# NethermindEth/latticefold

Measured on AMD Instinct MI355X. Metric: folding-prover steps/sec (one NIFSProver::prove per step), GoldilocksRingNTT, higher is better.
Workload: dtype u64; 1 GPU; C4: GoldilocksRingNTT R1CS->CCS, m=N=2^20 rows, wit_len=262144, L=4, B=2^16, b=2, K=16, kappa=26, t=3; parallelism=replicas x1

## Files before the change

latticefold_amd/csrc/lf_capi.cpp:

```cpp
#include "lf_ring_host.h"
#include <thread>
#include <vector>

const char *lf_strerror(int code) {
    switch (code) {
        case LF_OK: return "ok";
        case LF_ERR_INVALID: return "invalid argument / wrong length";
        case LF_ERR_HIP: return "HIP runtime error (no GPU or out of device memory)";
        case LF_ERR_UNSUPPORTED: return "unsupported parameter";
        case LF_ERR_BAD_TABLES: return "ring tables are not a ring isomorphism";
        case LF_ERR_NORM: return "witness coefficient exceeds the decomposition bound";
        case LF_ERR_SIZE_BOUNDS: return "invalid size bounds (m must be >= wit_len*L, power of two)";
        case LF_ERR_STATE: return "call sequence misuse";
        case LF_ERR_REJECT: return "verifier rejected the proof";
    }
    return "unknown error";
}
const char *lf_phase_name(int i) { return (i >= 0 && i < LF_N_PHASES) ? PHASE_NAMES[i] : ""; }

static int install_tables(lf_ctx *c, u64 nonres, const u64 *y) {
    CrtTables T;
    if (build_crt_tables(nonres, y, T) != 0) return LF_ERR_BAD_TABLES;
    c->ring.T = T;
    c->dcrt = make_dev_crt(T);
// ... 524 lines not shown
            return hipGetLastError() == hipSuccess ? LF_ERR_UNSUPPORTED : LF_ERR_HIP;
    }
    c->ev_end(ev);
    launch_crt_fwd(c->dcrt, coef, ntt, ne, c->stream());
    launch_soa_to_aos(ntt, out_dev, ne, c->stream());
    if (hipGetLastError() != hipSuccess) return LF_ERR_HIP;
    return LF_OK;
}
int sb_cut_parts(lf_ctx *c, const lf_witness *wit, const char *name, const unsigned char **D) {
    const lf_params &P = c->P;
    if (!sb_base_ok(P.b) || c->sh_world > 1 || c->comm[0].model) return LF_ERR_UNSUPPORTED;
    if (!sb_digits_cover(P.b, P.K, P.B, c->digit_mode)) return LF_ERR_UNSUPPORTED;
    unsigned char *d;
    const size_t ldn = sb_ld(c->N);
    RET(c->tbuf(name, (size_t)P.K * 24 * ldn, &d));
    if (launch_sb_cut(wit->planes, c->N, P.K, sb_log2(P.b), c->digit_mode, d, ldn, c->stream()) != 0) return LF_ERR_HIP;
    *D = d;
    return LF_OK;
}
int commit_download(lf_ctx *c, const u64 *dev, size_t words, u64 *host) {
    RET(exchange_modsum_dev(c, (u64 *)dev, words));
    return down_small(c, dev, words, host);
}
void shard_slice(const lf_ctx *c, size_t n, size_t *i0, size_t *cnt) {
    size_t per = (n + (size_t)c->sh_world - 1) / (size_t)c->sh_world;
    size_t lo = per * (size_t)c->sh_rank;
    if (lo > n) lo = n;
    *i0 = lo;
    *cnt = lo + per > n ? n - lo : per;
}
bool shard_keep(const lf_ctx *c, int kind, size_t n) {
    const size_t Gw = (size_t)c->sh_world;
    if (Gw <= 1 || n / 2 < Gw * 64) return false;
    size_t thr = kind ? c->tn.shard_fold_min : c->tn.shard_lin_min;
    if (thr > (c->m >> 4)) thr = c->m >> 4;
    return n > thr;
}
int gather_slices(lf_ctx *c, u64 *buf, size_t planes, size_t n) {
    const size_t Gw = (size_t)c->sh_world, lcl = n / Gw, words = planes * lcl;
    u64 *gall, *gtmp;
    RET(c->tbuf("sh_gather_tab", words * Gw, &gall));
    RET(c->tbuf("sh_gather_tmp", words, &gtmp));
    HIPCHK(hipMemcpy2DAsync(gtmp, lcl * 8, buf + (size_t)c->sh_rank * lcl, n * 8, lcl * 8, planes, hipMemcpyDeviceToDevice, c->stream()));
    RET(c->cm().allgather_dev(gtmp, gall, words, c->stream()));
    launch_gather_relayout(gall, (u32)Gw, planes, lcl, buf, c->stream());
    return LF_OK;
}
int gather_parts(lf_ctx *c, const GatherPart *parts, int np, size_t lcl) {
    const size_t Gw = (size_t)c->sh_world;
    size_t ptot = 0;
    for (int i = 0; i < np; i++) ptot += parts[i].planes;
    const size_t words = ptot * lcl;
    u64 *gall, *gtmp;
    RET(c->tbuf("sh_gather_tab", words * Gw, &gall));
    RET(c->tbuf("sh_gather_tmp", words, &gtmp));
    size_t p0 = 0;
    for (int i = 0; i < np; i++) {
        HIPCHK(hipMemcpy2DAsync(gtmp + p0 * lcl, lcl * 8, parts[i].src, parts[i].src_ld * 8, lcl * 8, parts[i].planes, hipMemcpyDeviceToDevice, c->stream()));
        p0 += parts[i].planes;
    }
    RET(c->cm().allgather_dev(gtmp, gall, words, c->stream()));
    p0 = 0;
    for (int i = 0; i < np; i++) {
        launch_gather_relayout_part(gall, (u32)Gw, ptot, p0, parts[i].planes, lcl, parts[i].dst, c->stream());
        p0 += parts[i].planes;
    }
    return LF_OK;
}
int lf_ajtai_commit(lf_ctx *c, const uint64_t *f, size_t n, size_t batch, uint64_t *out) {
    if (LF_XB(c) && f && out) {
        XB x(c, true);
        int rc = lf_ajtai_commit(c, f, n, batch, out);
        if (rc == LF_OK) x.ring_out(out, batch * c->core_any().kappa);
        return rc;
    }
    if (!c || !f || !out || !batch) return LF_ERR_INVALID;
    return c->bb ? ring_ops<BbRing>::ajtai_commit(c->bb->p, f, n, batch, out) : ring_ops<GoldRing>::ajtai_commit(c, f, n, batch, out);
}
int lf_ajtai_commit_dev(lf_ctx *c, const uint64_t *f, size_t n, size_t batch, uint64_t *out) {
    if (!c || !f || !out || !batch) return LF_ERR_INVALID;
    if (LF_XB(c)) {
        XB x(c, true);
        int rc = lf_ajtai_commit_dev(c, f, n, batch, out);
        if (rc == LF_OK) x.ring_out(out, batch * c->core_any().kappa);
        return rc;
    }
    return c->bb ? ring_ops<BbRing>::ajtai_commit(c->bb->p, f, n, batch, out, Origin::device) : ring_ops<GoldRing>::ajtai_commit(c, f, n, batch, out, Origin::device);
}
static int ajtai_commit_gadget_api(lf_ctx *c, const uint64_t *f, bool ntt_in, size_t count, bool dec, uint64_t base, unsigned digits, size_t batch, uint64_t *out,
                                   Origin org = Origin::host) {
    if (LF_XB(c) && f && out) {
        XB x(c, true);
        const u32 kap = c->core_any().kappa;
        int rc = ajtai_commit_gadget_api(c, f, ntt_in, count, dec, base, digits, batch, out, org);
        if (rc == LF_OK) x.ring_out(out, batch * kap);
        return rc;
    }
    if (!c || !f || !out || !batch || digits == 0 || digits > 64) return LF_ERR_INVALID;
    u32 lb = 0;
    if (dec) {
        if (!pow2(base) || (c->bb && base > (1ull << 32))) return LF_ERR_UNSUPPORTED;
        while ((1ull << lb) < base) lb++;
    }
    return c->bb ? ring_ops<BbRing>::ajtai_commit_gadget(c->bb->p, f, ntt_in, count, lb, digits, batch, out, org)
                 : ring_ops<GoldRing>::ajtai_commit_gadget(c, f, ntt_in, count, lb, digits, batch, out, org);
}
int lf_ajtai_commit_coeff(lf_ctx *c, const uint64_t *f_coeff, size_t n, size_t batch, uint64_t *out) {
    return ajtai_commit_gadget_api(c, f_coeff, false, n, false, 0, 1, batch, out);
}
int lf_ajtai_decompose_and_commit_coeff(lf_ctx *c, const uint64_t *f_coeff, size_t count, uint64_t base, unsigned digits, size_t batch, uint64_t *out) {
    return ajtai_commit_gadget_api(c, f_coeff, false, count, true, base, digits, batch, out);
}
int lf_ajtai_decompose_and_commit_ntt(lf_ctx *c, const uint64_t *w_ntt, size_t count, uint64_t base, unsigned digits, size_t batch, uint64_t *out) {
    return ajtai_commit_gadget_api(c, w_ntt, true, count, true, base, digits, batch, out);
}
int lf_ajtai_commit_coeff_dev(lf_ctx *c, const uint64_t *f_coeff, size_t n, size_t batch, uint64_t *out) {
    return ajtai_commit_gadget_api(c, f_coeff, false, n, false, 0, 1, batch, out, Origin::device);
}
int lf_ajtai_decompose_and_commit_coeff_dev(lf_ctx *c, const uint64_t *f_coeff, size_t count, uint64_t base, unsigned digits, size_t batch, uint64_t *out) {
    return ajtai_commit_gadget_api(c, f_coeff, false, count, true, base, digits, batch, out, Origin::device);
}
int lf_ajtai_decompose_and_commit_ntt_dev(lf_ctx *c, const uint64_t *w_ntt, size_t count, uint64_t base, unsigned digits, size_t batch, uint64_t *out) {
    return ajtai_commit_gadget_api(c, w_ntt, true, count, true, base, digits, batch, out, Origin::device);
}

int lf_modsum(const uint64_t *parts, size_t nparts, size_t words, uint64_t *out) {
    if (!parts || !out || !nparts) return LF_ERR_INVALID;
    for (size_t w = 0; w < words; w++) {
        u64 acc = 0;
        for (size_t g = 0; g < nparts; g++) {
            u64 v = parts[g * words + w];
            if (v >= LF_P) return LF_ERR_INVALID;
            acc = fq_add(acc, v);
        }
        out[w] = acc;
    }
    return LF_OK;
}
int lf_modsum_ring(const uint64_t *parts, size_t nparts, size_t words, uint64_t *out, int ring) {
    if (ring == LF_RING_GOLDILOCKS) return lf_modsum(parts, nparts, words, out);
    if (ring != LF_RING_BABYBEAR || !parts || !out || !nparts) return LF_ERR_INVALID;
    for (size_t w = 0; w < words; w++) {
        u64 acc = 0;
        for (size_t g = 0; g < nparts; g++) {
            u64 v = parts[g * words + w];
            if (v >= lfbb::BB_P) return LF_ERR_INVALID;
            acc += v;
        }
        out[w] = acc % lfbb::BB_P;
    }
    return LF_OK;
}

int build_eq_dev(lf_ctx *c, const Fq3 *pt, u32 nv, u64 *eq_dev) {
    Fq3Const *rd;
    RET(c->tbuf("eq_point", 64, &rd));
    std::vector<Fq3Const> h(nv);
    for (u32 i = 0; i < nv; i++) h[i] = f3c(pt[i]);
    RET(c->h2d_small(rd, h.data(), nv * sizeof(Fq3Const)));
    if (nv >= 6) {
        u64 *scr;
        RET(c->tbuf("eq_scratch", build_eq_scratch_words(nv), &scr));
        launch_build_eq2(c->dcrt, rd, nv, scr, eq_dev, c->stream());
    } else launch_build_eq(c->dcrt, rd, nv, eq_dev, c->stream());
    return LF_OK;
}
static int build_eq_api(lf_ctx *c, const uint64_t *point, unsigned nv, uint64_t *out, Origin org) {
    if (LF_XB(c) && point && out && nv && nv <= 40) {
        XB x(c, org == Origin::device);
        int rc = build_eq_api(c, x.ext_in(point, nv), nv, out, org);
        if (rc == LF_OK && org == Origin::host) x.ext_out(out, (size_t)1 << nv);
        return rc;
    }
    if (!c || !point || !out || nv == 0 || nv > 40) return LF_ERR_INVALID;
    return c->bb ? ring_ops<BbRing>::build_eq(c->bb->p, point, nv, out, org) : ring_ops<GoldRing>::build_eq(c, point, nv, out, org);
}
int lf_build_eq(lf_ctx *c, const uint64_t *point, unsigned nv, uint64_t *out) { return build_eq_api(c, point, nv, out, Origin::host); }
int lf_build_eq_dev(lf_ctx *c, const uint64_t *point, unsigned nv, uint64_t *out) { return build_eq_api(c, point, nv, out, Origin::device); }
static int mle_eval_batch_api(lf_ctx *c, const uint64_t *tables, size_t ntables, size_t len, const uint64_t *point, unsigned nv, uint64_t *out, Origin org) {
    if (LF_XB(c) && tables && point && out) {
        XB x(c, true);
        int rc = mle_eval_batch_api(c, tables, ntables, len, x.ext_in(point, nv), nv, out, org);
        if (rc == LF_OK) x.ring_out(out, ntables);
        return rc;
    }
    if (!c || !tables || !point || !out || !ntables || nv == 0 || nv > 40) return LF_ERR_INVALID;
    return c->bb ? ring_ops<BbRing>::mle_eval_batch(c->bb->p, tables, ntables, len, point, nv, out, org)
                 : ring_ops<GoldRing>::mle_eval_batch(c, tables, ntables, len, point, nv, out, org);
}
int lf_mle_eval_batch(lf_ctx *c, const uint64_t *tables, size_t ntables, size_t len, const uint64_t *point, unsigned nv, uint64_t *out) {
    return mle_eval_batch_api(c, tables, ntables, len, point, nv, out, Origin::host);
}
int lf_mle_eval_batch_dev(lf_ctx *c, const uint64_t *tables, size_t ntables, size_t len, const uint64_t *point, unsigned nv, uint64_t *out) {
    return mle_eval_batch_api(c, tables, ntables, len, point, nv, out, Origin::device);
}

size_t lf_lcccs_len_ring(const lf_params *p, int ring) { return lcccs_len(p, ring == LF_RING_BABYBEAR ? 9 : 3); }
size_t lf_cccs_len_ring(const lf_params *p, int) { return cccs_len(p); }
size_t lf_proof_len_ring(const lf_params *p, int ring) { return proof_len(p, ring == LF_RING_BABYBEAR ? 9 : 3); }
size_t lf_lcccs_len(const lf_params *p) { return lcccs_len(p, 3); }
size_t lf_cccs_len(const lf_params *p) { return cccs_len(p); }
size_t lf_proof_len(const lf_params *p) { return proof_len(p, 3); }

int lf_ccs_load(lf_ctx *c, const lf_params *p, const uint32_t *const *rowptr, const uint32_t *const *col, const uint64_t *const *val,
                const uint32_t *S_off, const uint32_t *S_idx, const uint64_t *cc) {
    if (LF_XB(c) && p && rowptr && col && val && S_off && S_idx && cc && p->t >= 1 && p->t <= 8 && p->s <= 30 && p->q <= 8) {
        XB x(c);
        const size_t m = (size_t)1 << p->s;
        const uint64_t *v2[8];
        for (u32 j = 0; j < p->t; j++) {
            if (!rowptr[j] || !val[j]) return LF_ERR_INVALID;
            v2[j] = x.ring_in(val[j], rowptr[j][m]);
        }
        return lf_ccs_load(c, p, rowptr, col, v2, S_off, S_idx, x.ring_in(cc, p->q));
    }
    if (!c || !p || !rowptr || !col || !val || !S_off || !S_idx || !cc) return LF_ERR_INVALID;
    if (c->bb) { RET(lfbb::ccs_envelope(p)); return ring_ops<BbRing>::ccs_load(c->bb->p, p, rowptr, col, val, S_off, S_idx, cc); }
    if (p->s < 3 || p->s > LF_S_MAX || p->t == 0 || p->t > 8 || p->q == 0 || p->q > 8 || p->K == 0 || p->K > 32 || p->L == 0 || p->L > 8 ||
        p->d > 7 || p->wit_len == 0)
        return LF_ERR_UNSUPPORTED;
    if (p->b != 2 && !sb_base_ok(p->b)) return LF_ERR_UNSUPPORTED;
    if (p->b != 2 && (c->sh_world > 1 || c->comm[0].model || p->K > 11)) return LF_ERR_UNSUPPORTED;
    if (!pow2(p->B) || p->B > (1ULL << 32)) return LF_ERR_UNSUPPORTED;
    if (!sb_digits_cover(p->b, p->K, p->B, c->digit_mode)) return LF_ERR_UNSUPPORTED;
    return ring_ops<GoldRing>::ccs_load(c, p, rowptr, col, val, S_off, S_idx, cc);
}
int lf_spmv(lf_ctx *c, unsigned j, const uint64_t *z, uint64_t *out) {
    XbArrays xa(c);
    if (!c || !z || !out) return LF_ERR_INVALID;
    return c->bb ? ring_ops<BbRing>::spmv(c->bb->p, j, z, out) : ring_ops<GoldRing>::spmv(c, j, z, out);
}
int lf_spmv_dev(lf_ctx *c, unsigned j, const uint64_t *z, uint64_t *out) {
    if (!c || !z || !out) return LF_ERR_INVALID;
    XbArrays xa(c);
    return c->bb ? ring_ops<BbRing>::spmv(c->bb->p, j, z, out, Origin::device) : ring_ops<GoldRing>::spmv(c, j, z, out, Origin::device);
}

struct lf_witness_job {
    std::future<int> fut;
    lf_witness *w = nullptr;
};
int lf_witness_from_w_ccs_begin(lf_ctx *c, const uint64_t *w_ccs, lf_witness_job **job) {
    if (!c || !w_ccs || !job) return LF_ERR_INVALID;
    if (!c->have_ccs_any()) return LF_ERR_STATE;
    lf_witness_job *j = new lf_witness_job();
    c->io_jobs.fetch_add(1);
    j->fut = std::async(std::launch::async, [c, w_ccs, j]() -> int {
        struct Done { lf_ctx *c; ~Done() { c->io_jobs.fetch_sub(1); } } done{c};
        if (c->bb || c->xb.on) return lf_witness_from_w_ccs(c, w_ccs, &j->w);
        std::lock_guard<std::mutex> g(c->io_mu);
        if (hipSetDevice(c->device) != hipSuccess) return LF_ERR_HIP;
        t_lane = 2;
        return ring_ops<GoldRing>::witness_from_w_ccs_lane(c, w_ccs, &j->w);
    });
    *job = j;
    return LF_OK;
}
int lf_witness_job_finish(lf_witness_job *job, lf_witness **out) {
    if (!job) return LF_ERR_INVALID;
    const int rc = job->fut.valid() ? job->fut.get() : LF_ERR_STATE;
    if (rc == LF_OK && out) *out = job->w;
    else if (job->w) lf_witness_free(job->w);
    delete job;
    return rc;
}
int lf_witness_from_w_ccs(lf_ctx *c, const uint64_t *w_ccs, lf_witness **out) {
    XbArrays xa(c);
    if (!c || !w_ccs || !out) return LF_ERR_INVALID;
    return c->bb ? ring_ops<BbRing>::witness_from_w_ccs(c->bb->p, w_ccs, out) : ring_ops<GoldRing>::witness_from_w_ccs(c, w_ccs, out);
}
int lf_witness_from_f_coeff(lf_ctx *c, const uint64_t *f_coeff, lf_witness **out) {
    if (!c || !f_coeff || !out) return LF_ERR_INVALID;
    return c->bb ? ring_ops<BbRing>::witness_from_f_coeff(c->bb->p, f_coeff, out) : ring_ops<GoldRing>::witness_from_f_coeff(c, f_coeff, out);
}
int lf_witness_from_f(lf_ctx *c, const uint64_t *f_ntt, lf_witness **out) {
    XbArrays xa(c);
    if (!c || !f_ntt || !out) return LF_ERR_INVALID;
    return c->bb ? ring_ops<BbRing>::witness_from_f(c->bb->p, f_ntt, out) : ring_ops<GoldRing>::witness_from_f(c, f_ntt, out);
}
int lf_witness_get_f_coeff(lf_ctx *c, const lf_witness *w, uint64_t *out) {
    if (!c || !w || !out || w->ctx != c) return LF_ERR_INVALID;
    return c->bb ? ring_ops<BbRing>::witness_get_f_coeff(c->bb->p, w, out) : ring_ops<GoldRing>::witness_get_f_coeff(c, w, out);
}
int lf_witness_get_f(lf_ctx *c, const lf_witness *w, uint64_t *out) {
    XbArrays xa(c);
    if (!c || !w || !out || w->ctx != c) return LF_ERR_INVALID;
    return c->bb ? ring_ops<BbRing>::witness_get_f(c->bb->p, w, out) : ring_ops<GoldRing>::witness_get_f(c, w, out);
}
int lf_witness_get_w_ccs(lf_ctx *c, const lf_witness *w, uint64_t *out) {
    XbArrays xa(c);
    if (!c || !w || !out || w->ctx != c) return LF_ERR_INVALID;
    return c->bb ? ring_ops<BbRing>::witness_get_w_ccs(c->bb->p, w, out) : ring_ops<GoldRing>::witness_get_w_ccs(c, w, out);
}
int lf_witness_from_w_ccs_dev(lf_ctx *c, const uint64_t *w_ccs, lf_witness **out) {
    if (!c || !w_ccs || !out) return LF_ERR_INVALID;
    XbArrays xa(c);
    return c->bb ? ring_ops<BbRing>::witness_from_w_ccs(c->bb->p, w_ccs, out, Origin::device) : ring_ops<GoldRing>::witness_from_w_ccs(c, w_ccs, out, Origin::device);
}
int lf_witness_from_f_coeff_dev(lf_ctx *c, const uint64_t *f_coeff, lf_witness **out) {
    if (!c || !f_coeff || !out) return LF_ERR_INVALID;
    XbArrays xa(c);
    return c->bb ? ring_ops<BbRing>::witness_from_f_coeff(c->bb->p, f_coeff, out, Origin::device) : ring_ops<GoldRing>::witness_from_f_coeff(c, f_coeff, out, Origin::device);
}
int lf_witness_from_f_dev(lf_ctx *c, const uint64_t *f_ntt, lf_witness **out) {
    if (!c || !f_ntt || !out) return LF_ERR_INVALID;
    XbArrays xa(c);
    return c->bb ? ring_ops<BbRing>::witness_from_f(c->bb->p, f_ntt, out, Origin::device) : ring_ops<GoldRing>::witness_from_f(c, f_ntt, out, Origin::device);
}
int lf_witness_get_f_coeff_dev(lf_ctx *c, const lf_witness *w, uint64_t *out) {
    if (!c || !w || !out || w->ctx != c) return LF_ERR_INVALID;
    XbArrays xa(c);
    return c->bb ? ring_ops<BbRing>::witness_get_f_coeff(c->bb->p, w, out, Origin::device) : ring_ops<GoldRing>::witness_get_f_coeff(c, w, out, Origin::device);
}
int lf_witness_get_f_dev(lf_ctx *c, const lf_witness *w, uint64_t *out) {
    if (!c || !w || !out || w->ctx != c) return LF_ERR_INVALID;
    XbArrays xa(c);
    return c->bb ? ring_ops<BbRing>::witness_get_f(c->bb->p, w, out, Origin::device) : ring_ops<GoldRing>::witness_get_f(c, w, out, Origin::device);
// ... 243 lines not shown
```

latticefold_amd/csrc/lf_ctx.h:

```cpp
#pragma once
#include <hip/hip_runtime.h>
#include <assert.h>
#include <string.h>

#include <atomic>
#include <chrono>
#include <condition_variable>
#include <functional>
#include <future>
#include <thread>
#include <map>
#include <memory>
#include <mutex>
#include <set>
#include <string>
#include <vector>

#include "../../include/lfhip.h"
#include "bb_capi.h"
#include "lf_ctx_core.h"
#include "lf_common.h"
#include "lf_dist.h"
#include "lf_kernels.h"
#include "lf_sb.h"
// ... 3 lines not shown

namespace lf {
void launch_fix_many(const DevCrt &t, const u64 *in, size_t ld_in, u64 *out, size_t ld_out, size_t n_in, u32 rows3, Fq3Const r, hipStream_t s);
}

#include <stdio.h>
#include <stdlib.h>
static bool lf_trace_on() { static int v = -1; if (v < 0) v = getenv("LF_TRACE") ? 1 : 0; return v == 1; }
#define LF_TRACE(c, msg)                                                              \
    do {                                                                              \
        if (lf_trace_on()) {                                                          \
            hipError_t e_ = hipStreamSynchronize((c)->stream());                            \
            fprintf(stderr, "[lf] %s:%d %s -> %s\n", __func__, __LINE__, msg, hipGetErrorString(e_)); \
            fflush(stderr);                                                           \
        }                                                                             \
    } while (0)

inline thread_local int t_lane = 0;

struct lf_transcript {
    Transcript t;
    lfbb::BbTranscript *bb = nullptr;
    lf_transcript() {}
    lf_transcript(const lf_transcript &o) : t(o.t), bb(o.bb ? new lfbb::BbTranscript(*o.bb) : nullptr) {}
    ~lf_transcript() { delete bb; }
};

struct Timeline {
    bool on;
    std::chrono::steady_clock::time_point t0;
    std::vector<std::pair<const char *, double>> marks, marks1;
    Timeline() : on(getenv("LF_TIMELINE") != nullptr), t0(std::chrono::steady_clock::now()) { marks1.reserve(32); }
    void mark(const char *what) {
        marks.push_back({what, std::chrono::duration<double, std::milli>(std::chrono::steady_clock::now() - t0).count()});
    }
    void mark1(const char *what) { marks1.push_back({what, std::chrono::duration<double, std::milli>(std::chrono::steady_clock::now() - t0).count()}); }
    void merge() {
        marks.insert(marks.end(), marks1.begin(), marks1.end());
        marks1.clear();
        std::stable_sort(marks.begin(), marks.end(), [](const std::pair<const char *, double> &a, const std::pair<const char *, double> &b) { return a.second < b.second; });
    }
    void dump() {
        if (!on) return;
        double prev = 0;
        for (auto &m : marks) { fprintf(stderr, "[timeline] %-28s at %8.3f ms  (+%7.3f)\n", m.first, m.second, m.second - prev); prev = m.second; }
    }
};
inline thread_local Timeline *t_tl = nullptr;
#define TL_MARK(x) do { if (t_tl) t_tl->mark(x); } while (0)
inline const char *tl_round_name(const char *what, unsigned round) {
    static std::mutex mu;
    static std::set<std::string> names;
    char nm[32];
    snprintf(nm, sizeof nm, "%s %u", what, round);
    std::lock_guard<std::mutex> g(mu);
    return names.insert(nm).first->c_str();
}
#define TL_MARK_ROUND(what, round) do { if (t_tl) t_tl->mark(tl_round_name(what, round)); } while (0)

static const char *PHASE_NAMES[LF_N_PHASES] = {"linearization", "decomp_crt_commit", "decomp_evals", "fold_prepare",
                                                "fold_sumcheck", "fold_finish", "host_transcript", "total"};

struct LaneWorker {
    std::thread th;
    std::mutex m;
    std::condition_variable cv;
    std::function<int()> job;
    bool has_job = false, done = false, stop = false;
    int rc = 0;
    void loop() {
        std::unique_lock<std::mutex> lk(m);
        for (;;) {
            cv.wait(lk, [&] { return has_job || stop; });
            if (stop) return;
            std::function<int()> j = std::move(job);
            has_job = false;
            lk.unlock();
            int r = j();
            lk.lock();
            rc = r;
            done = true;
            cv.notify_all();
        }
    }
    void submit(std::function<int()> j) {
        std::unique_lock<std::mutex> lk(m);
        if (!th.joinable()) th = std::thread([this] { loop(); });
        job = std::move(j);
        has_job = true;
        done = false;
        cv.notify_all();
    }
    int wait() {
        std::unique_lock<std::mutex> lk(m);
        cv.wait(lk, [&] { return done; });
        return rc;
    }
    ~LaneWorker() {
        {
            std::unique_lock<std::mutex> lk(m);
            stop = true;
            cv.notify_all();
        }
        if (th.joinable()) th.join();
    }
};

struct lf_ctx : CtxCore<u64> {
    lf_ctx() : CtxCore<u64>(8192, 2 * 9 * 24 * sizeof(u64)) {}
    int lane() const override { return t_lane; }
    lfbb::BbCtx *bb = nullptr;
    ExtBasis xb;
    hipStream_t &st_io = st_lane[2];
    std::mutex io_mu;
    std::atomic<int> io_jobs{0};
    inline CtxCoreBase &core_any();
    bool have_ccs_any() { return core_any().have_ccs; }
    const lf_params &params_any() { return core_any().P; }
    size_t n_any() { return core_any().n; }
    size_t m_any() { return core_any().m; }
    size_t N_any() { return core_any().N; }
    HostRing ring;
    DevCrt dcrt;
    LaneWorker lane1;
    int agreed_two_lanes = -1;
    bool two_lanes_ok = false;
    lfdist::Comm comm[2];
    lfdist::Comm &cm() { assert(t_lane < 2); return comm[t_lane]; }
    bool ccs_general = false;
    size_t shc_r0 = (size_t)-1, shc_rcnt = 0, shc_lo = 0, shc_hi = 0;
    LinCombDesc desc{};
    std::vector<std::pair<const char *, double>> tl_marks;
    const lf_witness *bits_wit[2] = {nullptr, nullptr};
    u32 *bits_ptr[2] = {nullptr, nullptr};
    hipEvent_t bits_ev[2] = {nullptr, nullptr};
    hipEvent_t ev_yR = nullptr, ev_yL = nullptr;
    u64 *h_pin2 = nullptr;
    size_t h_pin2_words = 0;
    int pin2(size_t words) {
        if (words <= h_pin2_words) return LF_OK;
        if (h_pin2) (void)hipHostFree(h_pin2);
        h_pin2 = nullptr; h_pin2_words = 0;
        if (hipHostMalloc((void **)&h_pin2, words * 8) != hipSuccess) return LF_ERR_HIP;
        h_pin2_words = words;
        return LF_OK;
    }
    hipStream_t st_aux = nullptr;
    hipEvent_t ev_aux = nullptr;
    u64 *h_aux = nullptr;
    unsigned lin_split_rounds = 0;

    unsigned char *stage[LF_NLANES] = {nullptr, nullptr, nullptr};
    size_t stage_off[LF_NLANES] = {0, 0, 0};
    static constexpr size_t STAGE_BYTES = (size_t)1 << 20;
    int h2d_small(void *dst, const void *src, size_t bytes) {
        unsigned char *&ring = stage[t_lane];
        if (!ring && hipHostMalloc((void **)&ring, STAGE_BYTES, hipHostMallocDefault) != hipSuccess) { ring = nullptr; return LF_ERR_HIP; }
        const size_t need = (bytes + 63) & ~(size_t)63;
        if (need > STAGE_BYTES) {
            HIPCHK(hipMemcpyAsync(dst, src, bytes, hipMemcpyHostToDevice, stream()));
            HIPCHK(hipStreamSynchronize(stream()));
            return LF_OK;
        }
        if (stage_off[t_lane] + need > STAGE_BYTES) {
            HIPCHK(hipStreamSynchronize(stream()));
            stage_off[t_lane] = 0;
        }
        unsigned char *slot = ring + stage_off[t_lane];
        stage_off[t_lane] += need;
        memcpy(slot, src, bytes);
        HIPCHK(hipMemcpyAsync(dst, slot, bytes, hipMemcpyHostToDevice, stream()));
        return LF_OK;
    }
    TailMail *tail_mail = nullptr;
    u32 *tail_counters = nullptr;
    u64 *tail_dev_chal = nullptr;
    u32 tail_epoch = 0;
    int num_cus = 0;
    int tail_setup() {
        if (tail_mail) return LF_OK;
        hipDeviceProp_t pr;
        HIPCHK(hipGetDeviceProperties(&pr, device));
        num_cus = pr.multiProcessorCount;
        void *d = nullptr;
        HIPCHK(lf_dev_malloc(&d, 4096));
        HIPCHK(hipMemset(d, 0, 4096));
        tail_counters = (u32 *)d;
        tail_dev_chal = (u64 *)((char *)d + 1024);
        HIPCHK(hipHostMalloc((void **)&tail_mail, sizeof(TailMail), hipHostMallocMapped | hipHostMallocCoherent));
        memset(tail_mail, 0, sizeof(TailMail));
        return LF_OK;
    }
    u64 *d_poseidon = nullptr;
    int poseidon_setup() {
        if (d_poseidon) return LF_OK;
        const u64 *a, *m;
        Transcript::params(&a, &m);
        HIPCHK(lf_dev_malloc(&d_poseidon, (720 + 576) * 8));
        HIPCHK(hipMemcpy(d_poseidon, a, 720 * 8, hipMemcpyHostToDevice));
        HIPCHK(hipMemcpy(d_poseidon + 720, m, 576 * 8, hipMemcpyHostToDevice));
        return LF_OK;
    }
    hipEvent_t ev_theta = nullptr;
    hipEvent_t ev_block = nullptr;
    int lane_sync() {
        if (t_lane == 1 && ev_block) {
            HIPCHK(hipEventRecord(ev_block, st_lane[1]));
            HIPCHK(hipEventSynchronize(ev_block));
            return LF_OK;
        }
        HIPCHK(hipStreamSynchronize(stream()));
        return LF_OK;
    }
};
inline CtxCoreBase &lf_ctx::core_any() { return bb ? bb->core() : *this; }


#pragma GCC visibility push(hidden)
Fq3Const f3c(Fq3 a);
bool shard_keep(const lf_ctx *c, int kind, size_t n);
int build_eq_dev(lf_ctx *c, const Fq3 *pt, u32 nv, u64 *eq_dev);
int exchange_modsum_dev(lf_ctx *c, u64 *inout_dev, size_t words);
int down_small(lf_ctx *c, const u64 *dsrc, size_t words, u64 *host);
void shard_slice(const lf_ctx *c, size_t n, size_t *i0, size_t *cnt);
struct GatherPart { const u64 *src; size_t src_ld; u64 *dst; size_t planes; };
int shard_col_range(lf_ctx *c, size_t r0, size_t rcnt, size_t *lo, size_t *hi);
int gather_slices(lf_ctx *c, u64 *buf, size_t planes, size_t n);
struct SideState {
    const int32_t *planes = nullptr;
    u64 *z = nullptr;
    u64 *eq_r = nullptr;
    std::vector<u64> lcccs;
    std::atomic<int> z_state{0};
    hipEvent_t z_ev = nullptr;
    const unsigned char *D = nullptr;
    u32 *sv_bits = nullptr;
    ~SideState() { if (z_ev) (void)hipEventDestroy(z_ev); }
};
int gather_parts(lf_ctx *c, const GatherPart *parts, int np, size_t lcl);
inline thread_local bool t_xb_active = false;
inline thread_local bool t_xb_arrays = false;
struct XB {
    lf_ctx *c;
    size_t RE, TAU;
    std::vector<std::unique_ptr<std::vector<u64>>> keep;
    lf_transcript *tr = nullptr;
    explicit XB(lf_ctx *cc, bool arrays = false) : c(cc), RE((size_t)lf_ring_words(lf_ctx_ring(cc))), TAU((size_t)lf_ring_tau(lf_ctx_ring(cc))) {
        t_xb_active = true;
        t_xb_arrays = arrays;
    }
    ~XB() {
        t_xb_active = false;
        t_xb_arrays = false;
        if (tr) { tr->t.set_basis(nullptr, nullptr); if (tr->bb) tr->bb->set_basis(nullptr, nullptr); }
    }
    const u64 *ring_in(const u64 *p, size_t elems) {
        if (!p) return p;
        keep.emplace_back(new std::vector<u64>(p, p + elems * RE));
        c->xb.to_int(keep.back()->data(), elems * 8);
        return keep.back()->data();
    }
    const u64 *ext_in(const u64 *p, size_t n) {
        if (!p) return p;
        keep.emplace_back(new std::vector<u64>(p, p + n * TAU));
        c->xb.to_int(keep.back()->data(), n);
        return keep.back()->data();
    }
    void ring_out(u64 *p, size_t elems) { if (p) c->xb.to_ext(p, elems * 8); }
    void ext_out(u64 *p, size_t n) { if (p) c->xb.to_ext(p, n); }
    void transcript(lf_transcript *t) {
        tr = t;
        if (t->bb) t->bb->set_basis(c->xb.T, c->xb.Ti);
        else t->t.set_basis(c->xb.T, c->xb.Ti);
    }
};
#define LF_XB(c) ((c) && (c)->xb.on && !t_xb_active)
struct XbArrays {
    const bool set;
    explicit XbArrays(lf_ctx *c) : set(LF_XB(c)) { if (set) t_xb_active = t_xb_arrays = true; }
    ~XbArrays() { if (set) t_xb_active = t_xb_arrays = false; }
};
int fold_impl(lf_ctx *c, Transcript &tr, SideState *S , u64 *lcccs_out, lf_witness **w_out, u64 *proof);
int commit_download(lf_ctx *c, const u64 *dev, size_t words, u64 *host);
int commit_parts_i8g(lf_ctx *c, const unsigned char *D, size_t ldn, u32 NP, u64 *out_dev);
int sb_cut_parts(lf_ctx *c, const lf_witness *wit, const char *name, const unsigned char **D);
int fold_impl_sb(lf_ctx *c, Transcript &tr, SideState *S , u64 *lcccs_out, lf_witness **w_out, u64 *proof);
struct FoldStep {
    lf_ctx *c;
    Transcript &tr;
    SideState *S;
    u64 *proof;
    const lf_params &P;
    const size_t m, n, N;
    const u32 K, K2, deg;
    const GoldV hv;
    std::vector<Fq3> alpha, zeta, mu, beta, pt;
    Fq3Const *d_mu = nullptr, *d_ap = nullptr, *d_zp = nullptr;
    u64 *G[2] = {nullptr, nullptr}, *eqb = nullptr, *zz = nullptr;
    FoldRoundArgs a;
    u64 *T5[2] = {nullptr, nullptr};
    const u64 *curF = nullptr;
    size_t ldF = 0;
    u64 *eq0 = nullptr, *q = nullptr, *dpart = nullptr, *d_theta = nullptr, *d_eta = nullptr;
    FoldStep(lf_ctx *c, Transcript &tr, SideState *S, u64 *proof);
    u64 *msg(u32 round) const { return proof + (size_t)(round - 1) * (deg + 1) * 24; }
    u64 *theta() const { return proof + (size_t)P.s * (deg + 1) * 24; }
    u64 *eta() const { return theta() + (size_t)K2 * 72; }
    int powers_alpha_zeta();
    int powers_mu();
    int prepare_buffers();
    int side_mz(int sd, hipStream_t st, u64 *zb, const char *zaos_name, size_t zc_lo, size_t zc_hi, size_t g_r0 = 0, size_t g_rcnt = (size_t)-1);
    void first_tables();
    void fix_special(u32 round, Fq3Const r, u64 *dst, hipStream_t sg);
    void set_tables(u64 *dst, size_t nn);
    int eval_buffers();
    int gather_q(hipStream_t s1f);
    int finish(u64 *lcccs_out, lf_witness **w_out, const std::function<int(const std::vector<int8_t> &rho8, int8_t *d_rho, int32_t *npl)> &fold_witness);
};
int sb_fold_round_abi(lf_ctx *c, const u64 *t5, const u64 *F, size_t n, const Fq3Const *d_mu, u64 *evals_out);
int dot_batch_dev(lf_ctx *c, const u64 *X, size_t ldx, u32 na, const u64 *Y, size_t ldy, u32 nb, size_t n, u64 *dpart, u64 *od, hipStream_t st = nullptr,
                         const char *tag = "", unsigned char *yb_pre = nullptr);
int coef_eval_dev(lf_ctx *c, const int32_t *planes, size_t n, const u64 *eq, size_t ldeq, u32 K, int mode_bits, u64 *partial, u64 *od, size_t ldp,
                         const lf_witness *wit = nullptr);
int lin_tail_rounds(lf_ctx *c, Transcript &tr, const u64 *cur, const u64 *cure, size_t n, u64 *tout, u64 *partial, u32 round, Fq3 *point,
                           u64 *msgs, u32 deg, const std::function<void(u32)> *after_round);
int build_z(lf_ctx *c, const int32_t *planes, u32 K, int mode_bits, const u64 *heads, u64 *z, size_t w0 = 0, size_t wcnt = (size_t)-1,
            const unsigned char *D = nullptr );
#pragma GCC visibility pop
```

latticefold_amd/csrc/lf_fold.cpp:

```cpp
#include "lf_ring_host.h"

static int tail_host_rounds(lf_ctx *c, Transcript &tr, u32 epoch, u32 nr, u32 npts, bool dev_transcript, u64 *msgs, Fq3 *pt,
                            const std::function<void(u32)> *after_round = nullptr, u32 round0 = 0) {
    TailMail *mail = c->tail_mail;
    const auto t_start = std::chrono::steady_clock::now();
    double host_us = 0, wait_us = 0;
    auto t_mark = t_start;
    const bool tl_on = t_tl && t_tl->on;
    for (u32 i = 0; i < nr; i++) {
        u32 spins = 0;
        while (__atomic_load_n(&mail->msg_seq[i], __ATOMIC_ACQUIRE) != epoch) {
            __builtin_ia32_pause();
            if ((++spins & 0xfff) == 0) {
                if (__atomic_load_n(&mail->err, __ATOMIC_RELAXED) == epoch ||
                    std::chrono::duration<double>(std::chrono::steady_clock::now() - t_start).count() > 10.0) {
                    __atomic_store_n(&mail->abort_seq, epoch, __ATOMIC_RELEASE);
                    (void)hipStreamSynchronize(c->stream());
                    return LF_ERR_HIP;
                }
            }
        }
        if (tl_on) { auto nw = std::chrono::steady_clock::now(); wait_us += std::chrono::duration<double, std::micro>(nw - t_mark).count(); t_mark = nw; }
        u64 *evs = msgs + (size_t)i * npts * 24;
        memcpy(evs, (const void *)mail->msg[i], (size_t)npts * 24 * 8);
        HostTimer ht(c);
        Fq3 r;
        if (dev_transcript) r = fq3_make(mail->chal_out[i][0], mail->chal_out[i][1], mail->chal_out[i][2]);
        else r = lfs::sumcheck_round<GoldV>(tr, evs, npts);
        pt[i] = r;
        if (i + 1 < nr && !dev_transcript) {
            mail->chal[i][0] = r.c[0]; mail->chal[i][1] = r.c[1]; mail->chal[i][2] = r.c[2];
            __atomic_store_n(&mail->chal_seq[i], epoch, __ATOMIC_RELEASE);
        }
        if (after_round) (*after_round)(round0 + i);
        if (tl_on) { auto nw = std::chrono::steady_clock::now(); host_us += std::chrono::duration<double, std::micro>(nw - t_mark).count(); t_mark = nw; }
    }
    if (dev_transcript) tr.set_state((const u64 *)mail->sponge);
    if (tl_on) fprintf(stderr, "[timeline]    tail: %u rounds, host transcript %.1f us, waiting for the GPU %.1f us\n", nr, host_us, wait_us);
    return LF_OK;
}
static int tail_sponge_to_device(lf_ctx *c, Transcript &tr, u64 **state_out) {
    RET(c->poseidon_setup());
    *state_out = c->tail_dev_chal + 4 * TAIL_MAX_ROUNDS;
    u64 st[26];
    tr.get_state(st);
    HIPCHK(hipMemcpyAsync(*state_out, st, sizeof(st), hipMemcpyHostToDevice, c->stream()));
    HIPCHK(hipStreamSynchronize(c->stream()));
    return LF_OK;
}
int lin_tail_rounds(lf_ctx *c, Transcript &tr, const u64 *cur, const u64 *cure, size_t n, u64 *tout, u64 *partial, u32 round, Fq3 *point,
                           u64 *msgs, u32 deg, const std::function<void(u32)> *after_round) {
    const lf_params &P = c->P;
    RET(c->tail_setup());
    LinTailArgs A;
    A.T = cur; A.E = cure; A.Tout = tout; A.n0 = n; A.rounds = P.s - round + 1; A.deg = deg; A.partial = partial;
    RET(c->tbuf("lin_tail_priv", lin_tail_priv_words(n, P.t), &A.priv));
    A.counters = c->tail_counters; A.dev_chal = c->tail_dev_chal;
    HIPCHK(hipHostGetDevicePointer((void **)&A.mail, c->tail_mail, 0));
    if (++c->tail_epoch >= (1u << 30)) c->tail_epoch = 1;
    A.epoch = c->tail_epoch;
    A.r_first = f3c(point[round - 2]);
    A.dev_transcript = (c->tn.device_transcript && !c->xb.on) ? 1u : 0u;
    A.pos_ark = A.pos_mds = nullptr; A.sponge_state = nullptr;
    if (A.dev_transcript) {
        RET(tail_sponge_to_device(c, tr, &A.sponge_state));
        A.pos_ark = c->d_poseidon; A.pos_mds = c->d_poseidon + 720;
    }
    if (launch_lin_tail(c->dcrt, c->desc, A, c->stream()) == 0) return LF_ERR_UNSUPPORTED;
    if (hipGetLastError() != hipSuccess) return LF_ERR_HIP;
    return tail_host_rounds(c, tr, A.epoch, A.rounds, deg + 1, A.dev_transcript != 0, msgs + (size_t)(round - 1) * (deg + 1) * 24, &point[round - 1], after_round, round);
}
static int fold_tail_rounds(lf_ctx *c, Transcript &tr, const FoldRoundArgs &a, u64 *curF, u64 *const Fbuf[2], u64 *T_other, const Fq3Const *d_mu,
                            u64 *partial, u32 round, std::vector<Fq3> &pt, u64 *msgs, u32 deg) {
    const lf_params &P = c->P;
    RET(c->tail_setup());
    const u32 nr = P.s - round + 1;
    FoldTailArgs A;
    A.T[0] = (u64 *)a.eqL; A.T[1] = T_other;
    A.F[0] = curF; A.F[1] = curF == Fbuf[0] ? Fbuf[1] : Fbuf[0];
    A.n0 = a.n; A.rounds = nr; A.K = P.K; A.mu_pow = d_mu; A.partial = partial;
    A.counters = c->tail_counters; A.dev_chal = c->tail_dev_chal;
    RET(c->tbuf("tail_eqpriv", fold_tail_eqpriv_words(a.n, P.K), &A.eqpriv));
    HIPCHK(hipHostGetDevicePointer((void **)&A.mail, c->tail_mail, 0));
    if (++c->tail_epoch >= (1u << 30)) c->tail_epoch = 1;
    A.epoch = c->tail_epoch;
    A.r_first = f3c(pt[round - 2]);
    A.dev_transcript = (c->tn.device_transcript && !c->xb.on) ? 1u : 0u;
    A.pos_ark = A.pos_mds = nullptr; A.sponge_state = nullptr;
    if (A.dev_transcript) {
        RET(tail_sponge_to_device(c, tr, &A.sponge_state));
        A.pos_ark = c->d_poseidon; A.pos_mds = c->d_poseidon + 720;
    }
    if (launch_fold_tail(c->dcrt, A, c->num_cus, c->stream()) == 0) return LF_ERR_UNSUPPORTED;
    if (hipGetLastError() != hipSuccess) return LF_ERR_HIP;
    return tail_host_rounds(c, tr, A.epoch, nr, deg + 1, A.dev_transcript != 0, msgs + (size_t)(round - 1) * (deg + 1) * 24, &pt[round - 1]);
}

FoldStep::FoldStep(lf_ctx *c_, Transcript &tr_, SideState *S_, u64 *proof_)
    : c(c_), tr(tr_), S(S_), proof(proof_), P(c_->P), m(c_->m), n(c_->n), N(c_->N), K(c_->P.K), K2(2 * c_->P.K), deg(2 * c_->P.b), hv{c_->ring}, pt(c_->P.s) {}
int FoldStep::powers_alpha_zeta() {
    std::vector<Fq3Const> a_pow((size_t)K2 * 3), z_pow((size_t)K2 * P.t);
    for (u32 i = 0; i < K2; i++) {
        lfs::powers(hv, alpha[i], 3, [&](u32 d, const Fq3 &pw) { a_pow[(size_t)i * 3 + d] = f3c(pw); });
        lfs::powers(hv, zeta[i], P.t, [&](u32 j, const Fq3 &pw) { z_pow[(size_t)i * P.t + j] = f3c(pw); });
    }
    RET(upload_consts(c, "c_ap", a_pow, &d_ap));
    return upload_consts(c, "c_zp", z_pow, &d_zp);
}
int FoldStep::powers_mu() {
    std::vector<Fq3Const> mu_pow((size_t)K2 * 3);
    for (u32 i = 0; i < K2; i++) lfs::powers(hv, mu[i], 3, [&](u32 d, const Fq3 &pw) { mu_pow[(size_t)i * 3 + d] = f3c(pw); });
    return upload_consts(c, "c_mu", mu_pow, &d_mu);
}
int FoldStep::prepare_buffers() {
    RET(c->tbuf("fold_G1", 24 * m, &G[0]));
    RET(c->tbuf("fold_G2", 24 * m, &G[1]));
    RET(c->tbuf("fold_eqb", 3 * m, &eqb));
    return c->tbuf("fold_zz", (size_t)P.t * 24 * n, &zz);
}
int FoldStep::side_mz(int sd, hipStream_t st, u64 *zb, const char *zaos_name, size_t zc_lo, size_t zc_hi, size_t g_r0, size_t g_rcnt) {
    launch_lincomb_z(c->dcrt, S[sd].z + zc_lo, n, K, d_zp + (size_t)sd * K * P.t, P.t, zc_hi - zc_lo, zb + zc_lo, st);
    if (c->ccs_general) {
        u64 *zaos;
        RET(c->tbuf(zaos_name, (size_t)P.t * n * 24, &zaos));
        launch_spmv_rows(c->dcrt, P.t, c->d_rowptr.data(), c->d_col.data(), c->d_val.data(), zb, (size_t)24 * n, n, zaos, G[sd], m, 0, st, g_r0, g_rcnt);
    } else
        launch_spmv_sum(c->dcrt, P.t, c->d_rowptr.data(), c->d_col.data(), c->d_val.data(), zb, (size_t)24 * n, n, G[sd], m, st, g_r0, g_rcnt);
    return LF_OK;
}
void FoldStep::first_tables() {
    a.eqL = S[0].eq_r; a.eqR = S[1].eq_r; a.eqB = eqb; a.G1 = G[0]; a.G2 = G[1]; a.ld = m; a.n = m;
    a.p0 = 0; a.pcnt = m / 2; a.pF0 = 0;
}
void FoldStep::set_tables(u64 *dst, size_t nn) {
    a.eqL = dst; a.eqR = dst + 3 * nn; a.eqB = dst + 6 * nn; a.G1 = dst + 9 * nn; a.G2 = dst + 33 * nn;
    a.ld = nn; a.n = nn;
}
void FoldStep::fix_special(u32 round, Fq3Const r, u64 *dst, hipStream_t sg) {
    const size_t nn = a.n / 2;
    if (round == 2) {
        launch_fix_many(c->dcrt, a.eqL, a.ld, dst, nn, a.n, 1, r, sg);
        launch_fix_many(c->dcrt, a.eqR, a.ld, dst + 3 * nn, nn, a.n, 1, r, sg);
        launch_fix_many(c->dcrt, a.eqB, a.ld, dst + 6 * nn, nn, a.n, 1, r, c->stream());
        launch_fix_many(c->dcrt, a.G1, a.ld, dst + 9 * nn, nn, a.n, 8, r, sg);
        launch_fix_many(c->dcrt, a.G2, a.ld, dst + 33 * nn, nn, a.n, 8, r, sg);
    } else if (sg != c->stream()) {
        launch_fix_many(c->dcrt, a.eqL, a.ld, dst, nn, a.n, 2, r, sg);
        launch_fix_many(c->dcrt, a.eqB, a.ld, dst + 6 * nn, nn, a.n, 1, r, c->stream());
        launch_fix_many(c->dcrt, a.G1, a.ld, dst + 9 * nn, nn, a.n, 16, r, sg);
    } else {
        launch_fix_many(c->dcrt, a.eqL, a.ld, dst, nn, a.n, 19, r, c->stream());
    }
}
int FoldStep::eval_buffers() {
    u64 *fsm;
    RET(c->tbuf("fold_eq0", 3 * m, &eq0));
    RET(c->tbuf("dec_q", (size_t)P.t * 24 * n, &q));
    RET(c->tbuf("dot_partial", dot_partial_words(K, P.t), &dpart));
    RET(c->tbuf("fold_small", (size_t)K2 * 72 + (size_t)K2 * P.t * 24 + 64, &fsm));
    d_theta = fsm; d_eta = fsm + (size_t)K2 * 72;
    return build_eq_dev(c, pt.data(), P.s, eq0);
}
int FoldStep::gather_q(hipStream_t s1f) {
    size_t c0, cnt;
    shard_slice(c, n, &c0, &cnt);
    if (P.t > 1) RET(c->fork(c->stream(), s1f));
    for (u32 j = 0; j < P.t; j++)
        launch_spmv_t_eq(c->dcrt, c->d_colptr[j], c->d_rowidx[j], c->d_valT[j], eq0, m, q + (size_t)j * 24 * n, n, (j & 1) ? s1f : c->stream(), c0, cnt);
    if (P.t > 1) RET(c->join(s1f, c->stream()));
    return LF_OK;
}
int FoldStep::finish(u64 *lcccs_out, lf_witness **w_out, const std::function<int(const std::vector<int8_t> &, int8_t *, int32_t *)> &fold_witness) {
    std::vector<u64> rho_c, rho;
    std::vector<int8_t> rho8;
    {
        HostTimer ht(c);
        tr.absorb_ring(eta(), (size_t)K2 * P.t);
        lfs::draw_rho(hv, tr, K2, rho_c, rho, &rho8);
    }
    int8_t *d_rho;
    RET(c->tbuf("c_rho", (size_t)K2 * 24 + 64, &d_rho));
    int32_t *npl;
    RET(lf_planes_alloc(c, N * 24 * 4, &npl));
    RET(fold_witness(rho8, d_rho, npl));
    u64 *nf = nullptr, *nw = nullptr;
    const size_t nf_bytes = N * 24 * 8, nw_bytes = (size_t)P.wit_len * 24 * 8;
    RET(lf_planes_alloc(c, nf_bytes, (int32_t **)&nf));
    RET(lf_planes_alloc(c, nw_bytes, (int32_t **)&nw));
    launch_recompose_crt(c->dcrt, npl, N, (u32)N, 1, P.B, 1, 0, nf, N, 0, c->stream());
    launch_recompose_crt(c->dcrt, npl, N, P.wit_len, P.L, P.B, 1, 0, nw, P.wit_len, 0, c->stream());
    if (hipGetLastError() != hipSuccess) return LF_ERR_HIP;
    LF_TRACE(c, "fold_witness");
    TL_MARK("  eta absorbed, rho drawn, fold_witness enqueued");
    {
        HostTimer ht(c);
        const size_t ll = lf_lcccs_len(&P);
        lfs::fold_instance(hv, P, pt, theta(), eta(), rho_c.data(), rho.data(), [&](u32 i) { return &S[i / K].lcccs[(size_t)(i % K) * ll * 24]; }, lcccs_out);
    }
    TL_MARK("  folded instance on the host");
    HIPCHK(hipStreamSynchronize(c->stream()));
    *w_out = new lf_witness{c, npl, N, c->device, N * 24 * 4};
    (*w_out)->f_ntt = nf; (*w_out)->f_bytes = nf_bytes; (*w_out)->w_ccs = nw; (*w_out)->w_bytes = nw_bytes;
    TL_MARK(" rho + fold_witness");
    return LF_OK;
}
static void fold_tab_poly(const GoldV &hv, u32 round, const Fq3 &r1v, std::vector<u64> &poly) {
    const int nd = round == 1 ? 2 : 4, ncode = round == 1 ? 9 : 81;
    poly.assign((size_t)ncode * 12, 0);
    const Fq3 one = fq3_one();
    auto small = [&](int v) { return v == 0 ? fq3_zero() : (v > 0 ? (v == 1 ? one : fq3_add(one, one)) : (v == -1 ? fq3_neg(one) : fq3_neg(fq3_add(one, one)))); };
    for (int code = 0; code < ncode; code++) {
        int dg[4] = {0, 0, 0, 0}, cc = code;
        for (int b = 0; b < nd; b++, cc /= 3) dg[b] = cc % 3 - 1;
        Fq3 f0, f1;
        if (round == 1) { f0 = small(dg[0]); f1 = small(dg[1]); }
        else {
            f0 = fq3_add(small(dg[0]), hv.ext_mul(small(dg[1] - dg[0]), r1v));
            f1 = fq3_add(small(dg[2]), hv.ext_mul(small(dg[3] - dg[2]), r1v));
        }
        Fq3 df = fq3_sub(f1, f0), f0s = hv.ext_mul(f0, f0), dfs = hv.ext_mul(df, df);
        Fq3 t1 = hv.ext_mul(f0s, df), t2 = hv.ext_mul(f0, dfs);
        Fq3 q[4] = {fq3_sub(hv.ext_mul(f0s, f0), f0), fq3_sub(fq3_add(fq3_add(t1, t1), t1), df), fq3_add(fq3_add(t2, t2), t2), hv.ext_mul(dfs, df)};
        for (int e = 0; e < 4; e++)
            for (int w = 0; w < 3; w++) poly[(size_t)code * 12 + 3 * e + w] = q[e].c[w];
    }
}
struct FoldB2 : FoldStep {
    using FoldStep::FoldStep;
    const size_t Gw = (size_t)c->sh_world, gr = (size_t)c->sh_rank;
    bool sv_split = false, fr_split = false, fused = false, use_lut = false, use_r4tab = false, use_r5 = false, use_sv = false, sv_two_streams = false;
    bool sharded = false;
    int flip = 0, fmode = 0;
    const u64 *prevF = nullptr;
    size_t prevld = 0, ldEr = 0;
    u64 *svE[3] = {nullptr, nullptr, nullptr}, *svE_rest = nullptr;
    u32 svE_level = 1;
    lfs::SplitCoef<GoldV> sp{};
    bool split_now = false;
    const u64 *Er = nullptr;
    u64 *F[2] = {nullptr, nullptr}, *partial = nullptr, *od = nullptr, *od_host = nullptr, *od_shard = nullptr, *d_lut = nullptr;
    u32 *sv_bits[2] = {nullptr, nullptr};
    hipStream_t sv_g_stream = nullptr;

    u64 *svE_ptr(u32 l) const {
        if (l <= 3) return svE[l - 1];
        size_t off = 0;
        for (u32 q = 4; q < l; q++) off += 3 * (m >> q);
        return svE_rest + off;
    }
    void svE_ensure(u32 l) {
        for (; svE_level < l; svE_level++)
            launch_eq_pairsum(svE_ptr(svE_level), m >> svE_level, m >> (svE_level + 1), svE_ptr(svE_level + 1), m >> (svE_level + 1), c->stream());
    }
    int prepare(), rounds_begin(), tail_handoff(u32 round, bool *done), fix_tables(u32 round, u64 *dst, bool *gathered), choose_producer(u32 round);
    void decide_split(u32 round);
    int gemm_round(u32 round), dispatch(u32 round), collect(u32 round), rounds(), evaluations();
};

int FoldB2::prepare() {
    { HostTimer ht(c); lfs::draw_alpha_zeta<GoldV>(tr, K2, alpha, zeta); }
    size_t ph = c->ev_begin(13);
    RET(powers_alpha_zeta());
    RET(prepare_buffers());
    RET(c->tbuf("round_partial", round_partial_words(), &partial));
    od = od_host = c->round_out();
    if (!od) return LF_ERR_HIP;
    if (c->sh_world > 1) {
        RET(c->tbuf("fold_round_out", 5 * 24 + 8, &od_shard));
        od = od_shard;
    }
    const bool shard_tabs = shard_keep(c, 1, m);
    const size_t g_r0 = shard_tabs ? (size_t)c->sh_rank * (m / (size_t)c->sh_world) : 0, g_rcnt = shard_tabs ? m / (size_t)c->sh_world : (size_t)-1;
    size_t zc_lo = 0, zc_hi = n;
    if (shard_tabs) RET(shard_col_range(c, g_r0, g_rcnt, &zc_lo, &zc_hi));
    {
        hipStream_t s0 = c->stream(), s1 = (t_lane == 0) ? c->st_lane[1] : s0;
        u64 *zz1 = zz;
        if (s1 != s0) RET(c->tbuf("fold_zz1", (size_t)P.t * 24 * n, &zz1));
        RET(c->fork(s0, s1));
        for (int sd = 0; sd < 2; sd++) {
            hipStream_t st = sd ? s1 : s0;
            RET(side_mz(sd, st, sd ? zz1 : zz, sd ? "spmv_zaos_R" : "spmv_zaos_L", zc_lo, zc_hi, g_r0, g_rcnt));
            launch_add_fhat_comb(c->dcrt, S[sd].planes, N, K, d_ap + (size_t)sd * K * 3, G[sd], m, st, g_r0, g_rcnt);
        }
        RET(c->join(s1, s0));
    }
    { HostTimer ht(c); lfs::draw_mu_beta<GoldV>(tr, K2, P.s, mu, beta); }
    TL_MARK(" fold challenges");
    RET(powers_mu());
    RET(build_eq_dev(c, beta.data(), P.s, eqb));
    sv_split = !c->tn.fold_sv_no_split && P.s >= 4 && m >= 256;
    if (sv_split) {
        RET(c->tbuf("fold_svE1", 3 * (m / 2), &svE[0]));
        RET(c->tbuf("fold_svE2", 3 * (m / 4), &svE[1]));
        RET(c->tbuf("fold_svE3", 3 * (m / 8), &svE[2]));
        RET(build_eq_dev(c, beta.data() + 1, P.s - 1, svE[0]));
    }
    fr_split = sv_split && c->sh_world == 1 && c->dcrt.nu2p40 && !c->tn.fold_rounds_no_split;
    if (fr_split) RET(c->tbuf("fold_svE_rest", 3 * (m / 8) + 64, &svE_rest));
    LF_TRACE(c, "fold prepare");
    c->ev_end(ph);
    if (t_tl && t_tl->on) { (void)hipStreamSynchronize(c->stream()); TL_MARK(" fold prepare (synced)"); }
    return LF_OK;
}
int FoldB2::rounds_begin() {
    sharded = Gw > 1;
    fused = !c->tn.fold_unfused && (Gw == 1 || !c->tn.shard_plain_rounds);
    use_lut = fused && P.s >= 4 && m / 4 >= c->tn.lut_min && m / 4 >= 4 && !c->tn.fold_no_lut;
    use_r4tab = use_lut && c->dcrt.nu2p40 && !c->tn.fold_no_r4tab;
    use_r5 = use_r4tab && !c->tn.fold_no_r5tab && Gw == 1 && P.s >= 5 && (N & 3) == 0 && (c->tn.no_tail || m / 8 > c->tn.tail_n) && m / 32 >= c->tn.r5_min;
    const size_t half = m / 2, f0_ent = use_lut ? m / 16 : m / 4, f1_ent = use_r5 ? m / 32 : m / 8;
    RET(c->tbuf("fold_F0", (size_t)K2 * 3 * 24 * (f0_ent ? f0_ent : 1), &F[0]));
    RET(c->tbuf("fold_F1", (size_t)K2 * 3 * 24 * (f1_ent ? f1_ent : 1), &F[1]));
    RET(c->tbuf("fold_T0", 57 * (half ? half : 1), &T5[0]));
    RET(c->tbuf("fold_T1", 57 * (half / 2 ? half / 2 : 1), &T5[1]));
    first_tables();
    c->sv_round_mask = 0;
    c->fold_split_mask = 0;
    sv_two_streams = t_lane == 0 && Gw == 1;
    sv_g_stream = c->stream();
    use_sv = !c->tn.force_exchange && !c->tn.fold_no_sv && (Gw == 1 || !c->tn.shard_plain_rounds) && N <= m && (N & 3) == 0 && !c->tn.fold_tab_r1;
    return LF_OK;
}
int FoldB2::tail_handoff(u32 round, bool *done) {
    if (sharded || c->tn.no_tail || round < 5 || !curF || ldF != a.n || a.n > c->tn.tail_n || a.n < 4 || P.s - round + 1 > TAIL_MAX_ROUNDS) return LF_OK;
    int trc = fold_tail_rounds(c, tr, a, (u64 *)curF, F, T5[flip], d_mu, partial, round, pt, proof, deg);
    if (trc == LF_OK) {
        curF = (u64 *)curF == F[0] ? F[1] : F[0];
        ldF = 2;
        *done = true;
    }
    return trc == LF_ERR_UNSUPPORTED ? LF_OK : trc;
}
int FoldB2::fix_tables(u32 round, u64 *dst, bool *gathered) {
    const Fq3Const r = f3c(pt[round - 2]);
    const size_t nn = a.n / 2;
    const bool handover = sharded && !shard_keep(c, 1, nn);
    hipStream_t sg = c->stream();
    if (use_sv && sv_two_streams && !sharded && (int)round <= c->tn.sv_rounds && round <= 3 && nn / 2 >= c->tn.sv_min && sv_shape_ok(1 << (round - 1), nn / 2, K))
        sg = c->st_lane[1];
    sv_g_stream = sg;
    if (!sharded) { fix_special(round, r, dst, sg); return LF_OK; }
    const size_t j0 = gr * (nn / Gw), jc = nn / Gw;
    if (round == 2) {
        launch_fix_many(c->dcrt, a.eqL + 2 * j0, a.ld, dst + j0, nn, 2 * jc, 1, r, sg);
        launch_fix_many(c->dcrt, a.eqR + 2 * j0, a.ld, dst + 3 * nn + j0, nn, 2 * jc, 1, r, sg);
        launch_fix_many(c->dcrt, a.eqB + 2 * j0, a.ld, dst + 6 * nn + j0, nn, 2 * jc, 1, r, sg);
        launch_fix_many(c->dcrt, a.G1 + 2 * j0, a.ld, dst + 9 * nn + j0, nn, 2 * jc, 8, r, sg);
        launch_fix_many(c->dcrt, a.G2 + 2 * j0, a.ld, dst + 33 * nn + j0, nn, 2 * jc, 8, r, sg);
    } else {
        launch_fix_many(c->dcrt, a.eqL + 2 * j0, a.ld, dst + j0, nn, 2 * jc, 19, r, sg);
    }
    if (!handover) return LF_OK;
    sharded = false;
    if (round <= 3) return gather_slices(c, dst, 57, nn);
    u64 *fd = F[(round & 1) ? 0 : 1];
    const size_t lcl = ldF / 2;
    launch_fix_many(c->dcrt, curF, ldF, fd, lcl, ldF, K2 * 3 * 8, r, c->stream());
    const GatherPart gp[2] = {{dst + gr * lcl, nn, dst, 57}, {fd, lcl, fd, (size_t)K2 * 3 * 24}};
    RET(gather_parts(c, gp, 2, lcl));
    curF = fd; ldF = nn;
    *gathered = true;
    return LF_OK;
}
int FoldB2::choose_producer(u32 round) {
    const size_t nn = a.n / 2;
    if (round == 3) {
        const size_t q = sharded ? nn / Gw : nn, j0 = sharded ? gr * q : 0;
        if (use_lut) {
            Fq3 lut[162];
            lfs::fold_lut81(hv, pt[0], pt[1], lut);
            RET(c->tbuf("fold_lut", 2 * 81 * 3 + 8, &d_lut));
            RET(c->h2d_small(d_lut, lut, sizeof(lut)));
            fmode = 3;
            curF = nullptr; ldF = q;
        } else {
            Fq3 Wf[4];
            lfs::eq_weights(hv, pt.data(), 2, Wf);
            const Fq3Const W[4] = {f3c(Wf[0]), f3c(Wf[1]), f3c(Wf[2]), f3c(Wf[3])};
            launch_fold_materialize2(c->dcrt, S[0].planes, S[1].planes, N, j0, q, K, W, F[0], c->stream());
            curF = F[0]; ldF = q;
        }
    } else if (round > 3) {
        u64 *fd = F[(round & 1) ? 0 : 1];
        if (use_lut && round == 4) fmode = 4;
        else if (use_r5 && round == 5) fmode = 7;
        else if (fused && ldF >= c->tn.fuse_min && ldF >= 4) { prevF = curF; prevld = ldF; fmode = 1; }
        else launch_fix_many(c->dcrt, curF, ldF, fd, ldF / 2, ldF, K2 * 3 * 8, f3c(pt[round - 2]), c->stream());
        curF = fd; ldF = ldF / 2;
    }
    return LF_OK;
}
void FoldB2::decide_split(u32 round) {
    Er = nullptr; ldEr = 0; split_now = false;
    if (!(fr_split && round >= 2 && !sharded && (fmode == 7 || (fmode == 4 && use_r4tab)) && a.pcnt >= c->tn.fold_split_min)) return;
    sp = lfs::split_coef(hv, lfs::eq_prefix(hv, beta.data(), pt.data(), round), beta[round - 1]);
    if (!sp.ok) return;
    svE_ensure(round);
    Er = svE_ptr(round); ldEr = m >> round;
    split_now = true;
    c->fold_split_mask |= 1u << (round - 1);
}
int FoldB2::gemm_round(u32 round) {
    const int svV = 1 << (round - 1);
    std::vector<Fq3> W((size_t)svV), Cf;
    lfs::eq_weights(hv, pt.data(), round - 1, W.data());
    lfs::sv_coef(hv, svV, W.data(), sv_num_pairs(svV), [&](int i) { return sv_pair(svV, i); }, Cf);
    u64 *d_coef, *gtmp, *svtp;
    unsigned char *sveb;
    int32_t *svpart, *svtot;
    RET(c->tbuf("sv_coef", Cf.size() * 3 + 8, &d_coef));
    RET(c->tbuf("sv_gtmp", 128, &gtmp));
    RET(c->tbuf("sv_tp", sv_tp_words(K), &svtp));
    RET(c->tbuf("sv_eb", sv_eb_bytes(a.pcnt), &sveb));
    RET(c->tbuf("sv_part", sv_part_words(svV, a.pcnt, K), &svpart));
    RET(c->tbuf("sv_tot", sv_tot_words(svV, K), &svtot));
    RET(c->h2d_small(d_coef, Cf.data(), Cf.size() * sizeof(Fq3)));
    if (!sv_bits[0])
        for (int sd = 0; sd < 2; sd++) {
            if (S[sd].sv_bits) { sv_bits[sd] = S[sd].sv_bits; continue; }
            RET(c->tbuf(sd ? "sv_bits_R" : "sv_bits_L", sv_bits_words(N, K), &sv_bits[sd]));
            launch_sv_bits(S[sd].planes, N, N, K, sv_bits[sd], c->stream());
        }
    hipStream_t sg = round == 1 ? (sv_two_streams && !sharded ? c->st_lane[1] : c->stream()) : sv_g_stream;
    if (round == 1) RET(c->fork(c->stream(), sg));
    launch_fold_round_g(c->dcrt, a, partial, gtmp, sg);
    hipEvent_t g_ready = nullptr;
    if (sg != c->stream() && !(g_ready = c->join_mark(sg))) return LF_ERR_HIP;
    const u64 *Ei = nullptr;
    size_t ldE = 0;
    Fq3Const w01[2] = {};
    if (sv_split) {
        const Fq3 ci = lfs::eq_prefix(hv, beta.data(), pt.data(), round), bi = beta[round - 1];
        w01[0] = f3c(hv.ext_mul(ci, fq3_sub(fq3_one(), bi)));
        w01[1] = f3c(hv.ext_mul(ci, bi));
        svE_ensure(round);
        Ei = svE[round - 1]; ldE = m >> round;
    }
    if (launch_sv_round(c->dcrt, svV, sv_bits[0], sv_bits[1], N, a.eqB, a.ld, a.p0, a.pcnt, K, d_mu, d_coef, sveb, svpart, svtot, svtp, gtmp, od, c->stream(), g_ready,
                        Ei, ldE, w01) != 0)
        return LF_ERR_UNSUPPORTED;
    c->sv_round_mask |= 1u << (round - 1);
    return LF_OK;
}
int FoldB2::dispatch(u32 round) {
    const int32_t *pL = S[0].planes, *pR = S[1].planes;
    hipStream_t st = c->stream();
    if (use_sv && (int)round <= c->tn.sv_rounds && round <= 3 && a.pcnt >= c->tn.sv_min && sv_shape_ok(1 << (round - 1), a.pcnt, K) && (a.p0 * ((size_t)1 << (round - 1))) % 256 == 0)
        return gemm_round(round);
    if ((round == 2 || (round == 1 && c->tn.fold_tab_r1)) && a.pcnt >= c->tn.tab_min) {
        std::vector<u64> poly;
        fold_tab_poly(hv, round, round == 2 ? pt[0] : fq3_zero(), poly);
        u64 *d_poly, *d_tp;
        RET(c->tbuf("fold_poly", 81 * 12 + 8, &d_poly));
        RET(c->tbuf("fold_tp", (size_t)K2 * 3 * 81 * 12, &d_tp));
        RET(c->h2d_small(d_poly, poly.data(), poly.size() * 8));
        launch_fold_round_tab(c->dcrt, (int)round, a, pL, pR, N, K, d_mu, d_poly, d_tp, partial, od, st);
        return LF_OK;
    }
    if (round == 1) launch_fold_round1(c->dcrt, a, pL, pR, N, K, d_mu, partial, od, st);
    else if (round == 2) launch_fold_round2(c->dcrt, a, pL, pR, N, K, d_mu, f3c(pt[0]), partial, od, st);
    else if (fmode == 3 && c->dcrt.nu2p40) {
        u64 *mutab;
        RET(c->tbuf("fold_mutab", (size_t)3 * K2 * 3 * 81 * 4, &mutab));
        launch_fold_round_lut_mu(c->dcrt, a, pL, pR, N, d_lut, mutab, K, d_mu, partial, od, st);
    } else if (fmode == 3) launch_fold_round_lut(c->dcrt, a, pL, pR, N, d_lut, K, d_mu, partial, od, st);
    else if (fmode == 4 && use_r4tab) {
        u64 *r4sq, *r4mt;
        RET(c->tbuf("fold_r4sq", (size_t)6561 * 4, &r4sq));
        RET(c->tbuf("fold_r4mt", (size_t)K2 * 3 * 162 * 4, &r4mt));
        launch_fold_round_lut_fix_tab(c->dcrt, a, pL, pR, N, d_lut, f3c(pt[round - 2]), r4sq, r4mt, use_r5 ? nullptr : (u64 *)curF, ldF, K, d_mu, partial, od, st, Er, ldEr);
    } else if (fmode == 7) {
        u64 *r5xx, *r5yy, *r5mt;
        RET(c->tbuf("fold_r5xx", (size_t)6561 * 4, &r5xx));
        RET(c->tbuf("fold_r5yy", (size_t)6561 * 4, &r5yy));
        RET(c->tbuf("fold_r5mt", (size_t)K2 * 3 * 324 * 4, &r5mt));
        launch_fold_round_lut_fix5(c->dcrt, a, pL, pR, N, d_lut, f3c(pt[round - 3]), f3c(pt[round - 2]), r5xx, r5yy, r5mt, (u64 *)curF, ldF, K, d_mu, partial, od, st, Er, ldEr);
    } else if (fmode == 4) launch_fold_round_lut_fix(c->dcrt, a, pL, pR, N, d_lut, f3c(pt[round - 2]), (u64 *)curF, ldF, K, d_mu, partial, od, st);
    else if (fmode == 1) launch_fold_round_fix(c->dcrt, a, prevF, prevld, f3c(pt[round - 2]), (u64 *)curF, ldF, K, d_mu, partial, od, st, Er, ldEr);
    else launch_fold_round(c->dcrt, a, curF, ldF, K, d_mu, partial, od, st);
    if (split_now) {
        u64 *partial_g;
        RET(c->tbuf("round_partial_g", round_partial_words(), &partial_g));
        launch_fold_round_g(c->dcrt, a, partial_g, od + 120, st);
    }
    return LF_OK;
}
int FoldB2::collect(u32 round) {
    if (od == od_shard) {
        if (sharded) RET(exchange_modsum_dev(c, od, (size_t)(deg + 1) * 24));
        HIPCHK(hipMemcpyAsync(od_host, od, (size_t)(deg + 1) * 24 * 8, hipMemcpyDeviceToHost, c->stream()));
    }
    return c->lane_sync();
}
int FoldB2::rounds() {
    size_t ph = c->ev_begin(14);
    { HostTimer ht(c); lfs::sumcheck_prologue<GoldV>(tr, P.s, deg); }
    RET(rounds_begin());
    for (u32 round = 1; round <= P.s; round++) {
        fmode = 0;
        bool done = false;
        RET(tail_handoff(round, &done));
        if (done) break;
        if (round > 1) {
            const size_t nn = a.n / 2;
            u64 *dst = T5[flip];
            bool gathered = false;
            RET(fix_tables(round, dst, &gathered));
            if (!gathered) RET(choose_producer(round));
            set_tables(dst, nn);
            flip ^= 1;
        }
        if (sharded && !shard_keep(c, 1, a.n)) sharded = false;
        if (sharded) { a.pcnt = a.n / 2 / Gw; a.p0 = gr * a.pcnt; a.pF0 = a.p0; }
        else { a.p0 = 0; a.pcnt = a.n / 2; a.pF0 = 0; }
        decide_split(round);
        size_t ev = c->ev_begin(0);
        RET(dispatch(round));
        c->ev_end(ev);
        LF_TRACE(c, "fold round");
        RET(collect(round));
        u64 *evs = msg(round);
        if (split_now) {
            HostTimer ht2(c);
            lfs::complete_fold_split(hv, sp, od_host, od_host + 120, msg(round - 1), pt[round - 2], evs);
        } else
            memcpy(evs, od_host, (size_t)(deg + 1) * 24 * 8);
        HostTimer ht(c);
        pt[round - 1] = lfs::sumcheck_round<GoldV>(tr, evs, deg + 1);
        if (round <= 3 || round == 6 || round == 10) TL_MARK_ROUND("  round", round);
    }
    TL_MARK(" fold sumcheck");
    c->ev_end(ph);
    return LF_OK;
}
int FoldB2::evaluations() {
    u64 *red;
    RET(c->tbuf("red_partial", 256 * 4096, &red));
    RET(eval_buffers());
    hipStream_t s1 = (t_lane == 0 && c->sh_world == 1 && c->st_lane[1]) ? c->st_lane[1] : c->stream();
    RET(gather_q(s1));
    RET(c->pin((size_t)K2 * 72 + (size_t)K2 * P.t * 24));
    u64 *hp = c->h_pin_ref();
    if (P.s >= 4 && curF && ldF == 2 && !c->tn.theta_eval) launch_fix_final(c->dcrt, curF, K2 * 3 * 8, f3c(pt[P.s - 1]), d_theta, c->stream());
    else {
        size_t i0, cnt;
        shard_slice(c, N, &i0, &cnt);
        for (int sd = 0; sd < 2; sd++) RET(coef_eval_dev(c, S[sd].planes + i0, cnt, eq0 + i0, m, K, 1, red, d_theta + (size_t)sd * K * 72, N));
        RET(exchange_modsum_dev(c, d_theta, (size_t)K2 * 72));
    }
    HIPCHK(hipMemcpyAsync(hp, d_theta, (size_t)K2 * 72 * 8, hipMemcpyDeviceToHost, c->stream()));
    if (!c->ev_theta) HIPCHK(hipEventCreateWithFlags(&c->ev_theta, hipEventDisableTiming));
    HIPCHK(hipEventRecord(c->ev_theta, c->stream()));
    {
        size_t c0, cnt;
        shard_slice(c, n, &c0, &cnt);
        if (s1 != c->stream()) {
            unsigned char *ybq = nullptr;
            if (!c->tn.dot_valu && cnt >= c->tn.dot_min && P.t <= 3 && K <= 16 && ((((size_t)(S[0].z + c0)) ^ ((size_t)(S[1].z + c0))) & 15) == 0) {
                RET(c->tbuf("dot_yb", dot_i8_yb_bytes(n + 1), &ybq));
                if (launch_dot_pack_y(S[0].z + c0, q + c0, n, P.t, cnt, ybq, c->stream()) != 0) ybq = nullptr;
            }
            RET(c->fork(c->stream(), s1));
            u64 *dpart1;
            RET(c->tbuf("dot_partial1", dot_partial_words(K, P.t), &dpart1));
            RET(dot_batch_dev(c, S[1].z + c0, n, K, q + c0, n, P.t, cnt, dpart1, d_eta + (size_t)K * P.t * 24, s1, "_1", ybq));
            if (!c->join_mark(s1)) return LF_ERR_HIP;
            RET(dot_batch_dev(c, S[0].z + c0, n, K, q + c0, n, P.t, cnt, dpart, d_eta, nullptr, "", ybq));
            RET(c->join_wait(c->stream()));
        } else
            for (int sd = 0; sd < 2; sd++) RET(dot_batch_dev(c, S[sd].z + c0, n, K, q + c0, n, P.t, cnt, dpart, d_eta + (size_t)sd * K * P.t * 24));
        RET(exchange_modsum_dev(c, d_eta, (size_t)K2 * P.t * 24));
    }
    HIPCHK(hipMemcpyAsync(hp + (size_t)K2 * 72, d_eta, (size_t)K2 * P.t * 24 * 8, hipMemcpyDeviceToHost, c->stream()));
    HIPCHK(hipEventSynchronize(c->ev_theta));
    memcpy(theta(), hp, (size_t)K2 * 72 * 8);
    {
        HostTimer ht(c);
        tr.absorb_ring(theta(), (size_t)K2 * 3);
    }
    HIPCHK(hipStreamSynchronize(c->stream()));
    memcpy(eta(), hp + (size_t)K2 * 72, (size_t)K2 * P.t * 24 * 8);
    TL_MARK(" theta/eta");
    return LF_OK;
}
int fold_impl(lf_ctx *c, Transcript &tr, SideState *S , u64 *lcccs_out, lf_witness **w_out, u64 *proof) {
    if (c->P.b != 2) return fold_impl_sb(c, tr, S, lcccs_out, w_out, proof);
    FoldB2 f(c, tr, S, proof);
    RET(f.prepare());
    RET(f.rounds());
    size_t ph = c->ev_begin(15);
    RET(f.evaluations());
    RET(f.finish(lcccs_out, w_out, [&](const std::vector<int8_t> &rho8, int8_t *d_rho, int32_t *npl) -> int {
        HIPCHK(hipMemcpyAsync(d_rho, rho8.data(), rho8.size(), hipMemcpyHostToDevice, c->stream()));
        LF_TRACE(c, "theta/eta");
        launch_fold_witness(S[0].planes, S[1].planes, f.N, f.K, d_rho, npl, c->stream());
        return LF_OK;
    }));
    c->ev_end(ph);
    return LF_OK;
}

// ... 123 lines not shown
```

latticefold_amd/csrc/lf_kernels.h:

```cpp
#pragma once
#include "lf_ajtai_i8.h"
#include "lf_sv_rounds.h"
#include <hip/hip_runtime.h>

#include "lf_host.h"

namespace lf {

struct DevCrt {
    u64 nu;
    int nu2p40;
    u64 w4, w2, w10, w1, w7, w5, w11;
    int slot_of_pos[8], pos1[8], pos2[8];
    u64 tw1[8], tw2[8];
};
DevCrt make_dev_crt(const CrtTables &T);

struct Fq3Const { u64 c[3]; };

struct XbMat3 { u64 m[9]; };
void launch_aos_to_soa(const u64 *aos, u64 *soa, size_t n, hipStream_t s, u32 *flag = nullptr, const XbMat3 *Ti = nullptr);
void launch_soa_to_aos(const u64 *soa, u64 *aos, size_t n, hipStream_t s, const u32 *unless_flag = nullptr, const XbMat3 *T = nullptr);
void launch_ext_to_aos(const u64 *soa, u64 *aos, size_t n, hipStream_t s, const XbMat3 *T = nullptr);
void launch_slot_const_check(const u64 *tab, size_t n, u32 *flag, hipStream_t s);
void launch_fill_uniform(u64 *dst, size_t words, u64 seed, size_t start, hipStream_t s);
void launch_fill_ajtai(u64 *A, u32 kappa, size_t n, size_t n_total, size_t col0, u64 seed, hipStream_t s, u32 row0 = 0);

void launch_modsum(const u64 *parts, u32 nparts, size_t words, u64 *out, hipStream_t s);
void launch_gather_relayout(const u64 *all, u32 nranks, size_t planes, size_t lcl, u64 *full, hipStream_t s);
void launch_gather_relayout_part(const u64 *all, u32 nranks, size_t planes_tot, size_t p0, size_t planes, size_t lcl, u64 *full, hipStream_t s);

constexpr u32 SELFTEST_OUT = 13, SELFTEST_OUTC = 12;
void launch_selftest_field(const u64 *in, u32 n, u32 nc, u64 nu_gen, u64 *out, u64 *outc, u64 *mism_dev, hipStream_t s);

void launch_crt_fwd(const DevCrt &t, const u64 *coef, u64 *ntt, size_t n, hipStream_t s);
void launch_icrt_dense(const u64 *icrt_mat , const u64 *ntt, u64 *coef, size_t n, hipStream_t s);
void launch_ring_mul_ntt(const DevCrt &t, const u64 *a, const u64 *b, size_t n_terms, size_t n, u64 *out, hipStream_t s, u32 *flag = nullptr, const XbMat3 *Ti = nullptr);
void launch_ring_mul_coeff(const DevCrt &t, const u64 *icrt_mat , const u64 *a, const u64 *b, size_t n_terms, size_t n, u64 *out, hipStream_t s);


void launch_decompose(const u64 *coef, size_t n, u64 base, u32 digits, int layout, u64 *out, hipStream_t s, int mode = 0);
void launch_recompose(const u64 *in, size_t n_out, u64 base, u32 digits, u64 *out, hipStream_t s);
void launch_coef_to_i32(const u64 *coef, int32_t *planes, size_t n, u32 bound, int *viol, hipStream_t s);
void launch_i32_to_coef(const int32_t *planes, u64 *coef, size_t n, hipStream_t s);
void launch_recompose_crt(const DevCrt &t, const int32_t *planes, size_t n_planes, u32 wit_len, u32 L, u64 B, u32 K,
                          int mode_bits, u64 *out, size_t ldz, size_t off, hipStream_t s);
void launch_linf(const u64 *coef, size_t n, u64 *out_max, hipStream_t s);


void launch_build_eq(const DevCrt &t, const Fq3Const *r_dev , u32 nv, u64 *eq , hipStream_t s);
size_t build_eq_scratch_words(u32 nv);
void launch_build_eq2(const DevCrt &t, const Fq3Const *r_dev, u32 nv, u64 *scratch, u64 *eq, hipStream_t s);
void launch_spmv(const DevCrt &t, const u32 *rowptr, const u32 *col, const u64 *val , const u64 *z,
                 size_t ldz, u64 *out, size_t m, int accumulate, hipStream_t s, size_t r0 = 0, size_t rcnt = (size_t)-1 );
void launch_spmv_sum(const DevCrt &t, u32 nm, const u32 *const *rowptr, const u32 *const *col, const u64 *const *val, const u64 *z,
                     size_t z_stride, size_t ldz, u64 *out, size_t m, hipStream_t s, size_t r0 = 0, size_t rcnt = (size_t)-1 );
void launch_spmv_rows(const DevCrt &t, u32 nm, const u32 *const *rowptr, const u32 *const *col, const u64 *const *val, const u64 *z, size_t z_stride, size_t n,
                      u64 *zaos, u64 *out, size_t m, int accumulate, hipStream_t s, size_t r0 = 0, size_t rcnt = (size_t)-1);
void launch_spmv_t_eq(const DevCrt &t, const u32 *colptr, const u32 *rowidx, const u64 *val, const u64 *eq, size_t m,
                      u64 *q, size_t n, hipStream_t s, size_t c0 = 0, size_t ccnt = (size_t)-1 );
void launch_dot_batch(const DevCrt &t, const u64 *X, size_t ldx, u32 na, const u64 *Y, size_t ldy, u32 nb, size_t n,
                      u64 *partial, u64 *out, hipStream_t s);
size_t dot_partial_words(u32 na, u32 nb);
void launch_dot_eq(const DevCrt &t, const u64 *X, size_t ldx, u32 na, const u64 *eq, size_t ldeq, size_t n, u64 *partial,
                   u64 *out, hipStream_t s);
void launch_coef_eval(const DevCrt &t, const int32_t *planes, size_t n, const u64 *eq, size_t ldeq, u32 K, int mode_bits,
                      u64 *partial, u64 *out, hipStream_t s, size_t ldp = 0);
size_t coef_eval_partial_words(u32 K);
void launch_lincomb_z(const DevCrt &t, const u64 *z, size_t ldz, u32 K, const Fq3Const *coef_dev , u32 tt, size_t n,
                      u64 *out, hipStream_t s, u32 per_slot = 0);
void launch_add_fhat_comb(const DevCrt &t, const int32_t *planes, size_t n_planes, u32 K, const Fq3Const *apow_dev ,
                          u64 *G, size_t m, hipStream_t s, size_t r0 = 0, size_t rcnt = (size_t)-1 );

void launch_fix_ring(const DevCrt &t, const u64 *in, u64 *out, size_t n_in, Fq3Const r, hipStream_t s);
void launch_fix_fq3(const DevCrt &t, const u64 *in, u64 *out, size_t n_in, Fq3Const r, hipStream_t s);
size_t dot_i8_yb_bytes(size_t n);
size_t dot_i8_part_words(size_t n);
size_t dot_i8_tot_words();
int launch_dot_batch_i8(const DevCrt &t, const u64 *X, size_t ldx, u32 na, const u64 *Y, size_t ldy, u32 nb, size_t n, unsigned char *YB, int32_t *part,
                        long long *tot, u64 *out, hipStream_t s, bool y_packed = false, u32 nb_out = 0, u32 b0 = 0);
int launch_dot_pack_y(const u64 *X, const u64 *Y, size_t ldy, u32 nb, size_t n, unsigned char *YB, hipStream_t s);
void launch_vs_combine(const u64 *vs , u32 K, u64 *v , hipStream_t s);
void launch_fix_final(const DevCrt &t, const u64 *in , u32 rows3, Fq3Const r, u64 *out , hipStream_t s);

struct LinCombDesc {
    u32 t, q;
    u32 S_off[9];
    u32 S_idx[16];
    u64 c[8][24];
    int c_unit[8];
    u32 first[8];
    u32 ms[8];
};
void launch_lin_round(const DevCrt &t, const LinCombDesc &desc, const u64 *mz, size_t ld, const u64 *eq, size_t ldeq, size_t n,
                      u32 deg, u64 *partial, u64 *out, hipStream_t s, u32 max_blocks = 0, u32 split_xmask = 0 );
void launch_lin_round_fused(const DevCrt &t, const LinCombDesc &desc, const u64 *mz_prev, size_t ld_prev, const u64 *eq_prev, size_t ldeq_prev, Fq3Const r, u64 *mz_out,
                            size_t ld_out, u64 *eq_out, size_t ldeq_out, size_t n, u32 deg, u64 *partial, u64 *out, hipStream_t s, u32 max_blocks = 0,
                            u32 split_xmask = 0 );
struct LinFix;
void launch_lin_round_wide(const DevCrt &t, const LinCombDesc &desc, const u64 *mz, size_t ld, const u64 *eq, size_t ldeq, size_t n, u32 deg, u64 *partial, u64 *out,
                           hipStream_t s, u32 max_blocks, u32 split_xmask, const LinFix *fx);
void launch_eq_pairsum(const u64 *in, size_t ld_in, size_t n_out, u64 *out, size_t ld_out, hipStream_t s);
void launch_eq_expand(const DevCrt &t, const u64 *E, size_t lde, size_t pairs, Fq3Const w0, Fq3Const w1, u64 *out, size_t ldo, hipStream_t s);

struct FoldRoundArgs {
    const u64 *eqL, *eqR, *eqB;
    const u64 *G1, *G2;
    size_t ld;
    size_t n;
    size_t p0, pcnt;
    size_t pF0;
};
void launch_fold_round1(const DevCrt &t, const FoldRoundArgs &a, const int32_t *planesL, const int32_t *planesR, size_t n_planes,
                        u32 K, const Fq3Const *mu_pow_dev , u64 *partial, u64 *out, hipStream_t s);
void launch_fold_round_g(const DevCrt &t, const FoldRoundArgs &a, u64 *partial, u64 *out, hipStream_t s);
void launch_fold_materialize(const DevCrt &t, const int32_t *planesL, const int32_t *planesR, size_t n_planes, size_t m, u32 K,
                             Fq3Const r1, u64 *F, hipStream_t s);
void launch_fold_round2(const DevCrt &t, const FoldRoundArgs &a, const int32_t *planesL, const int32_t *planesR, size_t n_planes, u32 K,
                        const Fq3Const *mu_pow_dev, Fq3Const r1, u64 *partial, u64 *out, hipStream_t s);
void launch_fold_round_tab(const DevCrt &t, int round, const FoldRoundArgs &a, const int32_t *planesL, const int32_t *planesR, size_t n_planes, u32 K,
                           const Fq3Const *mu_pow_dev, const u64 *poly_dev, u64 *tp_dev, u64 *partial, u64 *out, hipStream_t s);
void launch_fold_materialize2(const DevCrt &t, const int32_t *planesL, const int32_t *planesR, size_t n_planes, size_t j0, size_t q, u32 K,
                              const Fq3Const W[4], u64 *F, hipStream_t s);
void launch_fold_round(const DevCrt &t, const FoldRoundArgs &a, const u64 *F, size_t ldF, u32 K, const Fq3Const *mu_pow_dev,
                       u64 *partial, u64 *out, hipStream_t s);
void launch_fold_round_lut_fix_tab(const DevCrt &t, const FoldRoundArgs &a, const int32_t *planesL, const int32_t *planesR, size_t n_planes,
                                   const u64 *lut_dev, Fq3Const r, u64 *sq_dev, u64 *mt_dev, u64 *Fout, size_t ldout, u32 K, const Fq3Const *mu_pow_dev,
                                   u64 *partial, u64 *out, hipStream_t s, const u64 *E = nullptr, size_t ldE = 0 );
void launch_fold_round_lut_fix5(const DevCrt &t, const FoldRoundArgs &a, const int32_t *planesL, const int32_t *planesR, size_t n_planes,
                                const u64 *lut_dev, Fq3Const r3, Fq3Const r4, u64 *xx_dev, u64 *yy_dev, u64 *mt_dev, u64 *Fout, size_t ldout, u32 K,
                                const Fq3Const *mu_pow_dev, u64 *partial, u64 *out, hipStream_t s, const u64 *E = nullptr, size_t ldE = 0 );
void launch_fold_round_fix(const DevCrt &t, const FoldRoundArgs &a, const u64 *Fprev, size_t ldprev, Fq3Const r, u64 *Fout, size_t ldout, u32 K,
                           const Fq3Const *mu_pow_dev, u64 *partial, u64 *out, hipStream_t s, const u64 *E = nullptr, size_t ldE = 0 );
void launch_fold_round_lut(const DevCrt &t, const FoldRoundArgs &a, const int32_t *planesL, const int32_t *planesR, size_t n_planes,
                           const u64 *lut_dev, u32 K, const Fq3Const *mu_pow_dev, u64 *partial, u64 *out, hipStream_t s);
void launch_fold_round_lut_mu(const DevCrt &t, const FoldRoundArgs &a, const int32_t *planesL, const int32_t *planesR, size_t n_planes,
                              const u64 *lut_dev, u64 *mutab_dev, u32 K, const Fq3Const *mu_pow_dev, u64 *partial, u64 *out, hipStream_t s);
void launch_fold_round_lut_fix(const DevCrt &t, const FoldRoundArgs &a, const int32_t *planesL, const int32_t *planesR, size_t n_planes,
                               const u64 *lut_dev, Fq3Const r, u64 *Fout, size_t ldout, u32 K, const Fq3Const *mu_pow_dev, u64 *partial,
                               u64 *out, hipStream_t s);
size_t round_partial_words();

void launch_sponge_script(const u64 *ark, const u64 *mds, const u32 *ops, u32 nops, const u64 *words, u64 *out, u64 *state_out, hipStream_t s);

constexpr u32 TAIL_MAX_ROUNDS = 32;
struct TailMail {
    u64 msg[TAIL_MAX_ROUNDS][128];
    u32 msg_seq[TAIL_MAX_ROUNDS];
    u64 chal[TAIL_MAX_ROUNDS][4];
    u32 chal_seq[TAIL_MAX_ROUNDS];
    u32 abort_seq;
    u32 err;
    u64 chal_out[TAIL_MAX_ROUNDS][4];
    u64 sponge[32];
    u64 dbg[TAIL_MAX_ROUNDS][8];
};
struct FoldTailArgs {
    u64 *T[2];
    u64 *F[2];
    size_t n0;
    u32 rounds, K;
    const Fq3Const *mu_pow;
    u64 *partial;
    u64 *eqpriv;
    u32 *counters;
    u64 *dev_chal;
    TailMail *mail;
    u32 epoch;
    Fq3Const r_first;
    u32 dev_transcript;
    const u64 *pos_ark, *pos_mds;
    u64 *sponge_state;
};
struct LinTailArgs {
    const u64 *T;
    const u64 *E;
    u64 *Tout;
    size_t n0;
    u32 rounds, deg;
    u64 *partial;
    u64 *priv;
    u32 *counters;
    u64 *dev_chal;
    TailMail *mail;
    u32 epoch;
    Fq3Const r_first;
    u32 dev_transcript;
    const u64 *pos_ark, *pos_mds;
    u64 *sponge_state;
};
size_t lin_tail_priv_words(size_t n0, u32 t);
u32 launch_lin_tail(const DevCrt &t, const LinCombDesc &desc, const LinTailArgs &A, hipStream_t s);
constexpr u32 FOLD_TAIL_MAX_BLOCKS = 256;
size_t fold_tail_eqpriv_words(size_t n0, u32 K);
u32 launch_fold_tail(const DevCrt &t, const FoldTailArgs &A, int num_cus, hipStream_t s);

void launch_fold_witness(const int32_t *planesL, const int32_t *planesR, size_t n, u32 K, const int8_t *rho_dev, int32_t *out,
                         hipStream_t s);

}
```

latticefold_amd/csrc/lf_kernels.hip:

```cpp
#include "lf_kernels.h"

#include <stdlib.h>

#include "lf_kernels_dev.cuh"
#include "lf_sb.h"

namespace lf {


DevCrt make_dev_crt(const CrtTables &T) {
    DevCrt d;
    d.nu = T.nu; d.nu2p40 = T.nu_is_2p40;
    d.w4 = T.w4; d.w2 = T.w2; d.w10 = T.w10; d.w1 = T.w1; d.w7 = T.w7; d.w5 = T.w5; d.w11 = T.w11;
    for (int p = 0; p < 8; p++) {
        d.slot_of_pos[p] = T.slot_of_pos[p]; d.pos1[p] = T.pos1[p]; d.pos2[p] = T.pos2[p];
        d.tw1[p] = T.tw1[p]; d.tw2[p] = T.tw2[p];
    }
    return d;
}


__global__ void __launch_bounds__(256) k_modsum(const u64 *parts, u32 nparts, size_t words, u64 *out) {
    size_t w = (size_t)blockIdx.x * 256 + threadIdx.x;
    if (w >= words) return;
// ... 568 lines not shown
}
size_t coef_eval_partial_words(u32 K) { return (size_t)RED_BLOCKS * K * 72; }
void launch_coef_eval(const DevCrt &t, const int32_t *planes, size_t n, const u64 *eq, size_t ldeq, u32 K, int mode_bits, u64 *partial,
                      u64 *out, hipStream_t s, size_t ldp) {
    if (!ldp) ldp = n;
    u32 gb = (u32)((n + 255) / 256);
    if (gb > 64) gb = 64;
    if (gb < 1) gb = 1;
    static int kg = -1;
    if (kg < 0) kg = 8;
    if (mode_bits && kg == 16) hipLaunchKernelGGL(k_coef_eval<16>, dim3(gb, 24, (K + 15) / 16), dim3(256), 0, s, planes, ldp, n, eq, ldeq, K, mode_bits, partial);
    else if (mode_bits && kg == 8) hipLaunchKernelGGL(k_coef_eval<8>, dim3(gb, 24, (K + 7) / 8), dim3(256), 0, s, planes, ldp, n, eq, ldeq, K, mode_bits, partial);
    else hipLaunchKernelGGL(k_coef_eval<4>, dim3(gb, 24, mode_bits ? (K + 3) / 4 : 1), dim3(256), 0, s, planes, ldp, n, eq, ldeq, K, mode_bits, partial);
    hipLaunchKernelGGL(k_reduce_rows, dim3(K * 72), dim3(256), 0, s, partial, gb, K * 72, out);
}

template <bool NU, int TT, int TS = TT, int J0 = 0>
__global__ void __launch_bounds__(256) k_lincomb_z(DevCrt t, const u64 *z, size_t ldz, u32 K, const Fq3Const *coef, size_t n, u64 *out, u32 per_slot) {
    size_t i = (size_t)blockIdx.x * 256 + threadIdx.x;
    u32 slot = blockIdx.y;
    if (i >= n) return;
    LH5 acc[TT];
    Fq3 accg[TT];
#pragma unroll
    for (int j = 0; j < TT; j++) { lh5_zero(acc[j]); accg[j] = fq3_zero(); }
    auto cf = [&](u32 k, int j) {
        Fq3Const cc = coef[per_slot ? (size_t)(k * TS + J0 + j) * 8 + slot : (size_t)(k * TS + J0 + j)];
        return fq3_make(cc.c[0], cc.c[1], cc.c[2]);
    };
    u32 k = 0;
    if (NU) {
        for (; k + 3 < K; k += 4) {
            Fq3 x[4], cv[4];
#pragma unroll
            for (int q = 0; q < 4; q++) x[q] = ld3(z + (size_t)(k + q) * 24 * ldz, ldz, slot, i);
#pragma unroll
            for (int j = 0; j < TT; j++) {
#pragma unroll
                for (int q = 0; q < 4; q++) cv[q] = cf(k + q, j);
                lh5_macn<4>(acc[j], x, cv);
            }
        }
        for (; k + 1 < K; k += 2) {
            Fq3 x0 = ld3(z + (size_t)k * 24 * ldz, ldz, slot, i), x1 = ld3(z + (size_t)(k + 1) * 24 * ldz, ldz, slot, i);
#pragma unroll
            for (int j = 0; j < TT; j++) lh5_mac2(acc[j], x0, cf(k, j), x1, cf(k + 1, j));
        }
    }
    for (; k < K; k++) {
        Fq3 x = ld3(z + (size_t)k * 24 * ldz, ldz, slot, i);
#pragma unroll
        for (int j = 0; j < TT; j++) {
            Fq3 cv = cf(k, j);
            if (NU) lh5_mac(acc[j], x, cv);
            else accg[j] = fq3_add(accg[j], M3<NU>(x, cv, t.nu));
        }
    }
#pragma unroll
    for (int j = 0; j < TT; j++) st3(out + (size_t)(J0 + j) * 24 * ldz, ldz, slot, i, NU ? lh5_finish(acc[j]) : accg[j]);
}
void launch_lincomb_z(const DevCrt &t, const u64 *z, size_t ldz, u32 K, const Fq3Const *coef_dev, u32 tt, size_t n, u64 *out, hipStream_t s, u32 per_slot) {
    if (!n) return;
#define LF_LZ(N)                                                                                                                              \
    do {                                                                                                                                      \
        if (t.nu2p40) hipLaunchKernelGGL((k_lincomb_z<true, N>), dim3(cdiv(n, 256), 8), dim3(256), 0, s, t, z, ldz, K, coef_dev, n, out, per_slot);    \
        else hipLaunchKernelGGL((k_lincomb_z<false, N>), dim3(cdiv(n, 256), 8), dim3(256), 0, s, t, z, ldz, K, coef_dev, n, out, per_slot);            \
    } while (0)
    switch (tt) {
        case 1: LF_LZ(1); break;
        case 2: LF_LZ(2); break;
        case 3: LF_LZ(3); break;
        case 4: LF_LZ(4); break;
#define LF_LZ2(N, TS, J0)                                                                                                                     \
    do {                                                                                                                                      \
        if (t.nu2p40) hipLaunchKernelGGL((k_lincomb_z<true, N, TS, J0>), dim3(cdiv(n, 256), 8), dim3(256), 0, s, t, z, ldz, K, coef_dev, n, out, per_slot);    \
        else hipLaunchKernelGGL((k_lincomb_z<false, N, TS, J0>), dim3(cdiv(n, 256), 8), dim3(256), 0, s, t, z, ldz, K, coef_dev, n, out, per_slot);            \
    } while (0)
        case 5: LF_LZ2(4, 5, 0); LF_LZ2(1, 5, 4); break;
        case 6: LF_LZ2(4, 6, 0); LF_LZ2(2, 6, 4); break;
        case 7: LF_LZ2(4, 7, 0); LF_LZ2(3, 7, 4); break;
        case 8: LF_LZ2(4, 8, 0); LF_LZ2(4, 8, 4); break;
#undef LF_LZ2
        default: break;
    }
#undef LF_LZ
}

template <int NQ>
__global__ void __launch_bounds__(256) k_add_fhat_comb(const int32_t *planes, size_t n_planes, u32 K, const Fq3Const *apow, u64 *G, size_t m, size_t r0, size_t r1) {
    __shared__ u64 T[3 * NQ * 16][4];
    for (u32 e = threadIdx.x; e < 3 * NQ * 16; e += 256) {
        u32 val = e % 16, q = (e / 16) % NQ, d = e / (16 * NQ);
        Fq3 sum = fq3_zero();
        for (u32 b = 0; b < 4; b++)
            if (4 * q + b < K && ((val >> b) & 1)) {
                Fq3Const a = apow[(4 * q + b) * 3 + d];
                sum = fq3_add(sum, fq3_make(a.c[0], a.c[1], a.c[2]));
            }
        T[e][0] = sum.c[0]; T[e][1] = sum.c[1]; T[e][2] = sum.c[2]; T[e][3] = 0;
    }
    __syncthreads();
    size_t row = r0 + (size_t)blockIdx.x * 256 + threadIdx.x;
    u32 slot = blockIdx.y;
    if (row >= r1) return;
    Fq3 acc = ld3(G, m, slot, row);
#pragma unroll
    for (int d = 0; d < 3; d++) {
        int32_t v = planes[(size_t)(8 * d + slot) * n_planes + row];
        u32 mg = (u32)(v < 0 ? -v : v);
        Fq3 part = fq3_zero();
#pragma unroll
        for (int q = 0; q < NQ; q++) {
            const u64 *e = T[(d * NQ + q) * 16 + ((mg >> (4 * q)) & 15)];
            part = fq3_add(part, fq3_make(e[0], e[1], e[2]));
        }
        acc = v < 0 ? fq3_sub(acc, part) : fq3_add(acc, part);
    }
    st3(G, m, slot, row, acc);
}
void launch_add_fhat_comb(const DevCrt &t, const int32_t *planes, size_t n_planes, u32 K, const Fq3Const *apow_dev, u64 *G, size_t m,
                          hipStream_t s, size_t r0, size_t rcnt) {
    size_t r1 = rcnt == (size_t)-1 ? n_planes : (r0 + rcnt < n_planes ? r0 + rcnt : n_planes);
    if (rcnt == (size_t)-1) r0 = 0;
    if (r1 <= r0) return;
    if (K <= 16) hipLaunchKernelGGL(k_add_fhat_comb<4>, dim3(cdiv(r1 - r0, 256), 8), dim3(256), 0, s, planes, n_planes, K, apow_dev, G, m, r0, r1);
    else hipLaunchKernelGGL(k_add_fhat_comb<8>, dim3(cdiv(r1 - r0, 256), 8), dim3(256), 0, s, planes, n_planes, K, apow_dev, G, m, r0, r1);
}

template <bool NU>
__global__ void __launch_bounds__(256) k_fix(DevCrt t, const u64 *in, size_t ld_in, u64 *out, size_t ld_out, size_t n_out, Fq3Const r) {
    size_t j = (size_t)blockIdx.x * 256 + threadIdx.x;
    size_t row = blockIdx.y;
    if (j >= n_out) return;
    const u64 *p = in + row * 3 * ld_in;
    Fq3 rr = fq3_make(r.c[0], r.c[1], r.c[2]);
    ulonglong2 a0 = *(const ulonglong2 *)(p + 2 * j), a1 = *(const ulonglong2 *)(p + ld_in + 2 * j), a2 = *(const ulonglong2 *)(p + 2 * ld_in + 2 * j);
    Fq3 v0 = fq3_make(a0.x, a1.x, a2.x), v1 = fq3_make(a0.y, a1.y, a2.y);
    Fq3 res = fq3_add(v0, M3<NU>(fq3_sub(v1, v0), rr, t.nu));
    u64 *q = out + row * 3 * ld_out;
    q[j] = res.c[0]; q[ld_out + j] = res.c[1]; q[2 * ld_out + j] = res.c[2];
}
void launch_fix_ring(const DevCrt &t, const u64 *in, u64 *out, size_t n_in, Fq3Const r, hipStream_t s) {
    size_t n_out = n_in / 2;
    LF_LAUNCH(k_fix, t.nu2p40, dim3(cdiv(n_out, 256), 8), dim3(256), s, t, in, n_in, out, n_out, n_out, r);
}
void launch_fix_fq3(const DevCrt &t, const u64 *in, u64 *out, size_t n_in, Fq3Const r, hipStream_t s) {
    size_t n_out = n_in / 2;
    LF_LAUNCH(k_fix, t.nu2p40, dim3(cdiv(n_out, 256), 1), dim3(256), s, t, in, n_in, out, n_out, n_out, r);
}
void launch_fix_many(const DevCrt &t, const u64 *in, size_t ld_in, u64 *out, size_t ld_out, size_t n_in, u32 rows3, Fq3Const r, hipStream_t s) {
    size_t n_out = n_in / 2;
    LF_LAUNCH(k_fix, t.nu2p40, dim3(cdiv(n_out, 256), rows3), dim3(256), s, t, in, ld_in, out, ld_out, n_out, r);
}

template <bool NU>
__global__ void __launch_bounds__(256) k_fix_final(DevCrt t, const u64 *in, u32 rows3, Fq3Const r, u64 *out) {
    u32 row = blockIdx.x * 256 + threadIdx.x;
    if (row >= rows3) return;
    const u64 *p = in + (size_t)row * 6;
    Fq3 rr = fq3_make(r.c[0], r.c[1], r.c[2]);
    Fq3 v0 = fq3_make(p[0], p[2], p[4]), v1 = fq3_make(p[1], p[3], p[5]);
    Fq3 res = fq3_add(v0, M3<NU>(fq3_sub(v1, v0), rr, t.nu));
#pragma unroll
    for (int q = 0; q < 3; q++) out[(size_t)row * 3 + q] = fq_canon(res.c[q]);
}
__global__ void __launch_bounds__(128) k_vs_combine(const u64 *vs, u32 K, u64 *v) {
    const u32 i = threadIdx.x;
    if (i >= 72) return;
    u64 acc = 0, pw = 1;
    for (u32 k = 0; k < K; k++) {
        acc = fq_add(acc, fq_mul(fq_canon(vs[(size_t)k * 72 + i]), pw));
        pw = fq_add(pw, pw);
    }
    v[i] = fq_canon(acc);
}
void launch_vs_combine(const u64 *vs, u32 K, u64 *v, hipStream_t s) { hipLaunchKernelGGL(k_vs_combine, dim3(1), dim3(128), 0, s, vs, K, v); }
void launch_fix_final(const DevCrt &t, const u64 *in, u32 rows3, Fq3Const r, u64 *out, hipStream_t s) {
    LF_LAUNCH(k_fix_final, t.nu2p40, dim3(cdiv(rows3, 256)), dim3(256), s, t, in, rows3, r, out);
}

template <int NQ>
__global__ void __launch_bounds__(256) k_fold_witness(const int32_t *planesL, const int32_t *planesR, size_t n, u32 K, const int8_t *rho,
                                                      int32_t *out) {
    __shared__ __align__(16) int32_t R[2][2][NQ][16][28];
    lfk::fw_tables<NQ>(R, K, rho);
    __syncthreads();
    size_t j = (size_t)blockIdx.x * 256 + threadIdx.x;
    if (j >= n) return;
    int32_t win[31];
#pragma unroll
    for (int i = 0; i < 31; i++) win[i] = 0;
    lfk::fw_groups<0, 24, NQ>(win, planesL, planesR, n, j, R, out);
    int32_t delta[24];
#pragma unroll
    for (int i = 0; i < 24; i++) delta[i] = 0;
#pragma unroll
    for (int i = 22; i >= 12; i--) { win[i - 12] += win[i]; delta[i] -= win[i]; }
#pragma unroll
    for (int i = 11; i >= 0; i--) { delta[12 + i] += win[i]; delta[i] -= win[i]; }
#pragma unroll
    for (int c = 0; c < 24; c++) out[(size_t)c * n + j] += delta[c];
}
void launch_fold_witness(const int32_t *planesL, const int32_t *planesR, size_t n, u32 K, const int8_t *rho_dev, int32_t *out, hipStream_t s) {
    if (K <= 16) hipLaunchKernelGGL(k_fold_witness<4>, dim3(cdiv(n, 256)), dim3(256), 0, s, planesL, planesR, n, K, rho_dev, out);
    else hipLaunchKernelGGL(k_fold_witness<8>, dim3(cdiv(n, 256)), dim3(256), 0, s, planesL, planesR, n, K, rho_dev, out);
}

}
```

latticefold_amd/csrc/lf_sv_rounds.h:

```cpp
#pragma once
#include <hip/hip_runtime.h>
#include <stddef.h>
#include <stdint.h>
namespace lf {
struct SvPair {
    unsigned char s, b;
};
constexpr int sv_num_pairs(int V) { return 2 * V + 2 * V * (2 * V - 1) + 2 * V * (2 * V - 1) * (2 * V - 2) / 6; }
constexpr SvPair sv_pair(int V, int idx) {
    const int NX = 2 * V;
    int i = 0;
    for (int z = 0; z < NX; z++) {
        if (i == idx) return SvPair{(unsigned char)(1u << z), (unsigned char)(1u << z)};
        i++;
        for (int q = 0; q < NX; q++) {
            if (q == z) continue;
            if (i == idx) return SvPair{(unsigned char)(1u << z), (unsigned char)((1u << z) | (1u << q))};
            i++;
        }
    }
    for (int x = 0; x < NX; x++)
        for (int y = x + 1; y < NX; y++)
            for (int z = y + 1; z < NX; z++) {
                if (i == idx) {
                    const unsigned char m = (unsigned char)((1u << x) | (1u << y) | (1u << z));
                    return SvPair{m, m};
                }
                i++;
            }
    return SvPair{0, 0};
}
constexpr int sv_pairs_per_wave(int V, int NT = 3) { return V == 1 ? 4 : (V == 2 ? (NT == 2 ? 20 : 10) : (NT == 2 ? 40 : 20)); }

bool sv_shape_ok(int V, size_t npairs, uint32_t K);
size_t sv_eb_bytes(size_t npairs);
size_t sv_part_words(int V, size_t npairs, uint32_t K);
size_t sv_tot_words(int V, uint32_t K);
size_t sv_tp_words(uint32_t K);
size_t sv_bits_words(size_t n, uint32_t K, uint32_t rd = 24);
void launch_sv_bits(const int32_t *planes, size_t ldp, size_t n, uint32_t K, uint32_t *bits, hipStream_t s, uint32_t rd = 24);
size_t sv_tot_words_rd(uint32_t rd, int V, uint32_t K);
size_t sv_part_words_rd(uint32_t rd, int V, uint32_t K);
size_t sv_ldeb_pub(size_t npairs);
__host__ __device__ constexpr int sv_slot_pair_pub(int V, int j, int q) { return (j / (4 / V)) * (16 / V) + (j % (4 / V)) + (4 / V) * q; }
int launch_sv_gemm_tiles(uint32_t rd, int V, const uint32_t *bitsL, const uint32_t *bitsR, size_t nplanes, const unsigned char *EB, size_t ldeb, size_t npairs, uint32_t K,
                         int32_t *part, int32_t *tot, hipStream_t s);
struct DevCrt;
struct Fq3Const;
int launch_sv_round(const DevCrt &t, int V, const uint32_t *bitsL, const uint32_t *bitsR, size_t nplanes, const uint64_t *eqB, size_t ldeq, size_t pair0, size_t npairs, uint32_t K,
                    const Fq3Const *mu_pow, const uint64_t *coef, unsigned char *EB, int32_t *part, int32_t *tot, uint64_t *tp, const uint64_t *gpart, uint64_t *out,
                    hipStream_t s, hipEvent_t gpart_ready = nullptr,
                    const uint64_t *E = nullptr, size_t ldE = 0, const Fq3Const *w01 = nullptr);
size_t sv_vs_part_words(size_t n, uint32_t K);
size_t sv_vs_tot_words(uint32_t K);
int launch_sv_vs(const uint32_t *bits, size_t n, const uint64_t *eq, size_t ldeq, uint32_t K, unsigned char *EB, int32_t *part, int32_t *tot, uint64_t *out, hipStream_t s);
size_t sv_vs_max_blocks(uint32_t K);
size_t sv_vs_blocks_part_words(uint32_t nblocks, uint32_t K);
int launch_sv_vs_blocks(const uint32_t *bits, size_t n, const uint64_t *eq_lo, size_t ldeq, uint32_t J, uint32_t K, unsigned char *EB, int32_t *part, hipStream_t s);
void launch_sv_vs_combine(const DevCrt &t, const int32_t *part, uint32_t nblocks, const uint64_t *wts, uint32_t K, uint64_t *out, hipStream_t s);
}
```

latticefold_amd/csrc/lf_sv_rounds.hip:

```cpp
#include <hip/hip_runtime.h>
#include <cstdlib>
#include <utility>
#include "lf_field.cuh"
#include "lf_kernels.h"
#include "lf_sv_rounds.h"

namespace lf {
static inline size_t cdiv(size_t a, size_t b) { return (a + b - 1) / b; }
typedef int v4i __attribute__((ext_vector_type(4)));
constexpr u32 ONES4 = 0x01010101u;
constexpr int ctz8(unsigned m) { int i = 0; while (i < 8 && !((m >> i) & 1)) i++; return i; }
constexpr int pop8(unsigned m) { int n = 0; for (int i = 0; i < 8; i++) n += (m >> i) & 1; return n; }

__device__ __forceinline__ u32 sv_writelane(u32 val, u32 lane, u32 old) {
#if defined(__HIP_DEVICE_COMPILE__)
    asm("s_mov_b32 m0, %2\n\tv_writelane_b32 %0, %1, m0" : "+v"(old) : "s"(val), "s"(lane) : "m0");
    return old;
#else
    return old;
#endif
}
__global__ void __launch_bounds__(256) k_sv_bits(const int32_t *planes, size_t ldp, size_t n, size_t npad, u32 rows, u32 *bits, u32 rd) {
    const u32 lane = threadIdx.x & 63;
    const size_t wid = (size_t)blockIdx.x * 4 + (threadIdx.x >> 6), per_c = npad / 512;
    if (wid >= rd * per_c) return;
    const u32 c = (u32)(wid / per_c);
    const size_t base = (wid % per_c) * 512;
    u32 klo[8], khi[8];
#pragma unroll
    for (int it = 0; it < 8; it++) {
        const size_t pos = base + (size_t)it * 64 + lane;
        const int32_t v = pos < n ? planes[(size_t)c * ldp + pos] : 0;
        u32 m = v < 0 ? 0u - (u32)v : (u32)v;
        klo[it] = 0; khi[it] = 0;
        const unsigned long long sg = __ballot(v < 0);
        klo[it] = sv_writelane((u32)sg, rows - 1, klo[it]);
        khi[it] = sv_writelane((u32)(sg >> 32), rows - 1, khi[it]);
        for (u32 r = 0; r + 1 < rows; r++) {
            const unsigned long long bal = __ballot((int)(m & 1u));
            m >>= 1;
            klo[it] = sv_writelane((u32)bal, r, klo[it]);
            khi[it] = sv_writelane((u32)(bal >> 32), r, khi[it]);
        }
    }
    if (lane < rows) {
        u32 *o = bits + ((size_t)c * rows + lane) * (npad / 32) + base / 32;
#pragma unroll
        for (int it = 0; it < 8; it += 2) *(uint4 *)(o + 2 * it) = make_uint4(klo[it], khi[it], klo[it + 1], khi[it + 1]);
    }
}

__host__ __device__ constexpr int sv_slot_pair(int V, int j, int q) { return (j / (4 / V)) * (16 / V) + (j % (4 / V)) + (4 / V) * q; }

__global__ void __launch_bounds__(256) k_sv_pack_eq(const u64 *eq, size_t ld, size_t npairs, size_t ldeb, int V, unsigned char *EB, int single) {
    const size_t gid = (size_t)blockIdx.x * 256 + threadIdx.x, groups = ldeb / 16;
    if (gid >= groups * (single ? 3 : 6)) return;
    const u32 qh = (u32)(gid / groups), q = qh % 3, h = qh / 3;
    const size_t p0 = (gid % groups) * 16;
    u64 w[16];
#pragma unroll
    for (int t = 0; t < 16; t++) {
        const size_t pr = p0 + (size_t)sv_slot_pair(V, t >> 2, t & 3);
        const u64 e = pr < npairs ? (single ? eq[(size_t)q * ld + pr] : eq[(size_t)q * ld + 2 * pr + h]) : 0;
        u64 sb = e + 0x8080808080808080ull;
        if (sb < e) sb += 0xFFFFFFFFull;
        w[t] = sb ^ 0x8080808080808080ull;
    }
#pragma unroll
    for (int u = 0; u < 8; u++) {
        u32 o[4] = {0, 0, 0, 0};
#pragma unroll
        for (int t = 0; t < 16; t++) o[t >> 2] |= (u32)((w[t] >> (8 * u)) & 0xFF) << (8 * (t & 3));
        *(uint4 *)(EB + (size_t)(24 * h + 8 * q + u) * ldeb + p0) = make_uint4(o[0], o[1], o[2], o[3]);
    }
}

__device__ __forceinline__ u32 sv_full(u32 x) {
    u32 t, r;
    asm("v_lshlrev_b32 %0, 8, %1" : "=v"(t) : "v"(x));
    asm("v_sub_u32 %0, %1, %2" : "=v"(r) : "v"(t), "v"(x));
    return r;
}
struct SvGemmArgs {
    const u32 *bits[2];
    u32 rows;
    size_t nw;
    const unsigned char *EB;
    size_t ldeb;
    u32 ktiles;
    u32 nsides;
    u32 nsuper, super_per_chunk;
    u32 eb_mod;
    u32 rd;
    u32 super0;
    int32_t *part;
};

template <int V, int IDX>
__device__ __forceinline__ u32 sv_operand(const u32 (&Xf)[2 * V][4], const u32 (&S)[2 * V][4], const u32 (&D)[2 * V][4], int j) {
    constexpr SvPair pr = sv_pair(V, IDX);
    constexpr int nb = pop8(pr.b);
    if constexpr (nb == 1) {
        return D[ctz8(pr.b)][j];
    } else if constexpr (nb == 2) {
        constexpr int z = ctz8(pr.s), q = ctz8(pr.b & ~pr.s);
        return Xf[q][j] & D[z][j];
    } else {
        constexpr int x = ctz8(pr.b), y = ctz8(pr.b & ~(1u << x)), z = ctz8(pr.b & ~(1u << x) & ~(1u << y));
        return (Xf[x][j] & Xf[y][j] & Xf[z][j]) & ((S[x][j] ^ S[y][j] ^ S[z][j]) | ONES4);
    }
}
template <int V, int BASE, int I, int NT, bool VS>
__device__ __forceinline__ void sv_mfma_pair(v4i (&acc)[sv_pairs_per_wave(V, NT)][NT], const v4i (&b)[NT], const u32 (&Xf)[2 * V][4], const u32 (&S)[2 * V][4],
                                             const u32 (&D)[2 * V][4]) {
    if constexpr (VS && (I == 1 || I == 3)) return;
    v4i av;
    av.x = (int)sv_operand<V, BASE + I>(Xf, S, D, 0);
    av.y = (int)sv_operand<V, BASE + I>(Xf, S, D, 1);
    av.z = (int)sv_operand<V, BASE + I>(Xf, S, D, 2);
    av.w = (int)sv_operand<V, BASE + I>(Xf, S, D, 3);
#pragma unroll
    for (int nt = 0; nt < NT; nt++)
        if (!VS || (I == 0 && nt < 2) || (I == 2 && nt > 0)) acc[I][nt] = __builtin_amdgcn_mfma_i32_16x16x64_i8(av, b[nt], acc[I][nt], 0, 0, 0);
}
template <int V, int BASE, int NT, bool VS, int... I>
__device__ __forceinline__ void sv_mfma_all(v4i (&acc)[sv_pairs_per_wave(V, NT)][NT], const v4i (&b)[NT], const u32 (&Xf)[2 * V][4], const u32 (&S)[2 * V][4],
                                            const u32 (&D)[2 * V][4], std::integer_sequence<int, I...>) {
    (sv_mfma_pair<V, BASE, I, NT, VS>(acc, b, Xf, S, D), ...);
}

constexpr int sv_waves(int V) { return V <= 2 ? 8 : 4; }
template <int V, int PG, int NT = 3, bool VS = false>
__global__ void __launch_bounds__(64 * sv_waves(V)) __attribute__((amdgpu_waves_per_eu(V <= 2 ? 2 : 1, V <= 2 ? 2 : 1))) k_sv_gemm(SvGemmArgs a) {
    static_assert(!VS || (V == 1 && NT == 3 && PG == 0), "VS: the two single pairs of the round-1 shape");
    constexpr int NX = 2 * V, PW = sv_pairs_per_wave(V, NT), NPR = sv_num_pairs(V), SS = 4 / V, RPW = 4 / V;
    constexpr int NW = sv_waves(V), NTH = 64 * NW;
    constexpr int SPAIRS = 256 / V, LROW = SPAIRS + 16;
    constexpr int PIECES = 16 * NT * SPAIRS / 16, PPT = (PIECES + NTH - 1) / NTH;
    __shared__ __attribute__((aligned(16))) unsigned char lds[2][16 * NT][LROW];
    const u32 tid = threadIdx.x, lane = tid & 63, wave = tid >> 6, row = lane & 15, g = lane >> 4;
    const u32 ngroups = a.rd * a.nsides * a.ktiles, gq = ngroups / NW;
    const u32 grp = (blockIdx.x % gq) * NW + wave, chunk = blockIdx.x / gq;
    const u32 kt = grp % a.ktiles, c = (grp / a.ktiles) % a.rd, side = grp / (a.ktiles * a.rd);
    const u32 *mrow = a.bits[side] + ((size_t)c * a.rows + 16 * kt + row) * a.nw;
    const u32 *srow = a.bits[side] + ((size_t)c * a.rows + a.rows - 1) * a.nw;
    v4i acc[PW][NT];
#pragma unroll
    for (int i = 0; i < PW; i++)
#pragma unroll
        for (int nt = 0; nt < NT; nt++) acc[i][nt] = v4i{0, 0, 0, 0};
    const u32 u0 = chunk * a.super_per_chunk, u1 = u0 + a.super_per_chunk < a.nsuper ? u0 + a.super_per_chunk : a.nsuper;
    v4i st[PPT];
    auto stage_load = [&](u32 u) {
        const u32 ue = a.eb_mod ? u % a.eb_mod : u;
#pragma unroll
        for (int i = 0; i < PPT; i++) {
            const u32 t = tid + i * NTH;
            if (PIECES % NTH == 0 || t < PIECES) st[i] = *(const v4i *)(a.EB + (size_t)(t / (SPAIRS / 16)) * a.ldeb + (size_t)ue * SPAIRS + 16 * (t % (SPAIRS / 16)));
        }
    };
    auto stage_store = [&](u32 buf) {
#pragma unroll
        for (int i = 0; i < PPT; i++) {
            const u32 t = tid + i * NTH;
            if (PIECES % NTH == 0 || t < PIECES) *(v4i *)&lds[buf][t / (SPAIRS / 16)][16 * (t % (SPAIRS / 16))] = st[i];
        }
    };
    if (u0 < u1) { stage_load(u0); stage_store(0); }
    uint4 wm4 = make_uint4(0, 0, 0, 0), ws4 = wm4;
    mrow += (size_t)a.super0 * 16; srow += (size_t)a.super0 * 16;
    if (u0 < u1) { wm4 = *(const uint4 *)(mrow + ((size_t)u0 * 4 + g) * 4); ws4 = *(const uint4 *)(srow + ((size_t)u0 * 4 + g) * 4); }
    __syncthreads();
    for (u32 u = u0; u < u1; u++) {
        const u32 buf = (u - u0) & 1;
        const u32 wm[4] = {wm4.x, wm4.y, wm4.z, wm4.w}, wsg[4] = {ws4.x, ws4.y, ws4.z, ws4.w};
        const u32 un = u + 1 < u1 ? u + 1 : u;
        stage_load(un);
        wm4 = *(const uint4 *)(mrow + ((size_t)un * 4 + g) * 4);
        ws4 = *(const uint4 *)(srow + ((size_t)un * 4 + g) * 4);
#pragma unroll
        for (int ss = 0; ss < SS; ss++) {
            v4i b[NT];
            const unsigned char *lb = &lds[buf][row][g * (64 / V) + 16 * ss];
#pragma unroll
            for (int nt = 0; nt < NT; nt++) b[nt] = *(const v4i *)(lb + 16 * nt * LROW);
            u32 Xf[NX][4], S[NX][4], D[NX][4];
#pragma unroll
            for (int j = 0; j < 4; j++) {
                const u32 wmj = wm[ss * V + j / RPW], wsj = wsg[ss * V + j / RPW];
#pragma unroll
                for (int x = 0; x < NX; x++) {
                    const int sh = NX * (j % RPW) + x;
                    const u32 x1 = (wmj >> sh) & ONES4, s1 = (wsj >> sh) & ONES4;
                    Xf[x][j] = sv_full(x1);
                    S[x][j] = sv_full(s1);
                    D[x][j] = Xf[x][j] & (S[x][j] | ONES4);
                }
            }
            sv_mfma_all<V, PG * PW, NT, VS>(acc, b, Xf, S, D, std::make_integer_sequence<int, PW>{});
        }
        stage_store(buf ^ 1);
        __syncthreads();
    }
    int32_t *o = a.part + (((size_t)chunk * ngroups + grp) * NPR + (size_t)PG * PW) * (NT * 256);
#pragma unroll
    for (int i = 0; i < PW; i++)
#pragma unroll
        for (int nt = 0; nt < NT; nt++) *(v4i *)(o + ((size_t)i * NT + nt) * 256 + lane * 4) = acc[i][nt];
}

__global__ void __launch_bounds__(256) k_sv_sum(const int32_t *part, size_t words, u32 chunks, int32_t *tot) {
    const size_t i = ((size_t)blockIdx.x * 256 + threadIdx.x) * 4;
    if (i >= words) return;
    v4i s = v4i{0, 0, 0, 0};
    for (u32 ch = 0; ch < chunks; ch++) s += *(const v4i *)(part + (size_t)ch * words + i);
    *(v4i *)(tot + i) = s;
}

template <bool NU>
__global__ void __launch_bounds__(128) k_sv_finish1(DevCrt t, const int32_t *tot, u32 npr, u32 K, u32 ktiles, const u64 *coef, const Fq3Const *mu_pow, u64 *tp, u32 nt, Fq3Const w0,
                                                    Fq3Const w1) {
    const u32 T = blockIdx.x, c = T % 24, k = (T / 24) % K, side = T / (24 * K);
    const u32 grp = (side * 24 + c) * ktiles + k / 16, krow = k & 15;
    __shared__ u64 sm[15][128];
    const u32 pi = threadIdx.x;
    Fq3 P[5];
#pragma unroll
    for (int e = 0; e < 5; e++) P[e] = fq3_zero();
    if (pi < npr) {
        const int32_t *base = tot + ((size_t)grp * npr + pi) * (nt * 256);
        auto cell = [&](u32 bp) { return (long long)base[(bp >> 4) * 256 + ((bp & 15) + 16 * (krow >> 2)) * 4 + (krow & 3)]; };
        Fq3 M[2];
#pragma unroll
        for (int h = 0; h < 2; h++)
#pragma unroll
            for (int q = 0; q < 3; q++) {
                __int128 v = 0;
                if (nt == 3 || h == 0)
                    for (u32 u = 0; u < 8; u++) v += (__int128)cell(24 * h + 8 * q + u) << (8 * u);
                M[h].c[q] = fq_from_s128((u64)v, (int64_t)(v >> 64));
            }
        if (nt != 3) {
            const Fq3 Mp = M[0];
            M[0] = fq3_mul<NU>(Mp, fq3_make(w0.c[0], w0.c[1], w0.c[2]), t.nu);
            M[1] = fq3_mul<NU>(Mp, fq3_make(w1.c[0], w1.c[1], w1.c[2]), t.nu);
        }
        const Fq3 dM = fq3_sub(M[1], M[0]);
#pragma unroll
        for (int e = 0; e < 4; e++) {
            const u64 *cp = coef + ((size_t)pi * 4 + e) * 3;
            const Fq3 C = fq3_make(cp[0], cp[1], cp[2]);
            P[e] = fq3_add(P[e], fq3_mul<NU>(C, M[0], t.nu));
            P[e + 1] = fq3_add(P[e + 1], fq3_mul<NU>(C, dM, t.nu));
        }
    }
#pragma unroll
    for (int e = 0; e < 5; e++)
#pragma unroll
        for (int q = 0; q < 3; q++) sm[3 * e + q][threadIdx.x] = P[e].c[q];
    __syncthreads();
    if (threadIdx.x < 15) {
        u64 s = 0;
        for (u32 i = 0; i < 128; i++) s = fq_add(s, sm[threadIdx.x][i]);
        sm[threadIdx.x][0] = s;
    }
    __syncthreads();
    if (threadIdx.x < 5) {
        const u32 e = threadIdx.x;
        const Fq3Const mc = mu_pow[(side * K + k) * 3 + c / 8];
        const Fq3 r = fq3_mul<NU>(fq3_make(mc.c[0], mc.c[1], mc.c[2]), fq3_make(sm[3 * e][0], sm[3 * e + 1][0], sm[3 * e + 2][0]), t.nu);
#pragma unroll
        for (int q = 0; q < 3; q++) tp[((size_t)T * 5 + e) * 3 + q] = fq_canon(r.c[q]);
    }
}
__global__ void __launch_bounds__(1024) k_sv_finish2(const u64 *tp, u32 K, const u64 *gpart, u64 *out) {
    __shared__ u64 sm[8][128];
    const u32 i = threadIdx.x & 127, j = threadIdx.x >> 7;
    const u32 X = i / 24, slot = (i % 24) / 3, q = i % 3;
    u64 v = 0;
    if (i < 120) {
        u64 co[5] = {0, 0, 0, 0, 0};
        for (u32 sk = j; sk < 2 * K; sk += 8)
            for (u32 d = 0; d < 3; d++) {
                const u64 *p = tp + ((size_t)(sk * 24 + 8 * d + slot) * 5) * 3 + q;
#pragma unroll
                for (int e = 0; e < 5; e++) co[e] = fq_add(co[e], p[3 * e]);
            }
        v = co[4];
        for (int e = 3; e >= 0; e--) v = fq_add(fq_mul(v, (u64)X), co[e]);
    }
    sm[j][i] = v;
    __syncthreads();
    if (j == 0 && i < 120) {
        u64 s = fq_canon(gpart[i]);
#pragma unroll
        for (int w = 0; w < 8; w++) s = fq_add(s, sm[w][i]);
        out[i] = fq_canon(s);
    }
}

template <int V, int PG, int NT = 3>
void launch_gemm_pg(const SvGemmArgs &a, u32 grid, hipStream_t s) {
    hipLaunchKernelGGL((k_sv_gemm<V, PG, NT>), dim3(grid), dim3(64 * sv_waves(V)), 0, s, a);
    if constexpr (PG + 1 < sv_num_pairs(V) / sv_pairs_per_wave(V, NT)) launch_gemm_pg<V, PG + 1, NT>(a, grid, s);
}

bool sv_shape_ok(int V, size_t npairs, uint32_t K) {
    return (V == 1 || V == 2 || V == 4) && npairs >= 64 && npairs % 16 == 0 && npairs <= ((size_t)1 << 23) && K >= 1 && K <= 32;
}
static size_t sv_ldeb(size_t npairs) { return (npairs + 255) / 256 * 256; }
size_t sv_eb_bytes(size_t npairs) { return 48 * sv_ldeb(npairs) + 64; }
static size_t sv_npad(size_t n) { return (n + 511) / 512 * 512; }
size_t sv_bits_words(size_t n, uint32_t K, uint32_t rd) { return (size_t)rd * (16 * ((K + 15) / 16) + 1) * (sv_npad(n) / 32); }
void launch_sv_bits(const int32_t *planes, size_t ldp, size_t n, uint32_t K, uint32_t *bits, hipStream_t s, uint32_t rd) {
    const size_t npad = sv_npad(n);
    hipLaunchKernelGGL(k_sv_bits, dim3((unsigned)cdiv(rd * (npad / 512), 4)), dim3(256), 0, s, planes, ldp, n, npad, 16 * ((K + 15) / 16) + 1, bits, rd);
}
static uint32_t sv_chunks_n(int V, size_t nsuper, uint32_t K, uint32_t nsides, uint32_t rd = 24) {
    const u32 ktiles = (K + 15) / 16, per_chunk = rd * nsides * ktiles / (u32)sv_waves(V);
    if (nsuper == 0) return 1;
    size_t want = 256 / per_chunk;
    if (want > nsuper) want = nsuper;
    if (want < 1) want = 1;
    const size_t spc = cdiv(nsuper, want);
    return (u32)cdiv(nsuper, spc);
}
uint32_t sv_chunks(int V, size_t nsuper, uint32_t K) { return sv_chunks_n(V, nsuper, K, 2); }
size_t sv_tot_words(int V, uint32_t K) { return (size_t)48 * ((K + 15) / 16) * sv_num_pairs(V) * 768; }
static uint32_t sv_max_chunks(int V, uint32_t K, uint32_t nsides, uint32_t rd = 24) {
    const u32 per_chunk = rd * nsides * ((K + 15) / 16) / (u32)sv_waves(V);
    return per_chunk >= 256 ? 1 : 256 / per_chunk;
}
size_t sv_part_words(int V, size_t, uint32_t K) { return sv_tot_words(V, K) * sv_max_chunks(V, K, 2); }
size_t sv_tp_words(uint32_t K) { return (size_t)2 * K * 24 * 15; }

size_t sv_tot_words_rd(uint32_t rd, int V, uint32_t K) { return (size_t)2 * rd * ((K + 15) / 16) * sv_num_pairs(V) * 768; }
size_t sv_part_words_rd(uint32_t rd, int V, uint32_t K) { return sv_tot_words_rd(rd, V, K) * sv_max_chunks(V, K, 2, rd); }
size_t sv_ldeb_pub(size_t npairs) { return (npairs + 255) / 256 * 256; }
int launch_sv_gemm_tiles(uint32_t rd, int V, const uint32_t *bitsL, const uint32_t *bitsR, size_t nplanes, const unsigned char *EB, size_t ldeb, size_t npairs, uint32_t K,
                         int32_t *part, int32_t *tot, hipStream_t s) {
    if (!sv_shape_ok(V, npairs, K) || (2 * rd * ((K + 15) / 16)) % (u32)sv_waves(V)) return -1;
    const size_t wall = cdiv(nplanes, 2 * (size_t)V), wpairs = wall < npairs ? wall : npairs;
    SvGemmArgs a;
    a.bits[0] = bitsL; a.bits[1] = bitsR;
    a.ktiles = (K + 15) / 16;
    a.nsides = 2;
    a.rd = rd;
    a.rows = 16 * a.ktiles + 1;
    a.nw = sv_npad(nplanes) / 32;
    a.EB = EB; a.ldeb = ldeb;
    a.nsuper = (u32)cdiv(wpairs * V, 256);
    a.super0 = 0;
    a.eb_mod = 0;
    const u32 chunks = sv_chunks_n(V, a.nsuper, K, 2, rd);
    a.super_per_chunk = (u32)cdiv(a.nsuper, chunks);
    a.part = part;
    const u32 grid = 2 * rd * a.ktiles / (u32)sv_waves(V) * chunks;
    if (V == 1) launch_gemm_pg<1, 0>(a, grid, s);
    else if (V == 2) launch_gemm_pg<2, 0>(a, grid, s);
    else launch_gemm_pg<4, 0>(a, grid, s);
    const size_t words = sv_tot_words_rd(rd, V, K);
    hipLaunchKernelGGL(k_sv_sum, dim3((unsigned)cdiv(words / 4, 256)), dim3(256), 0, s, part, words, chunks, tot);
    return 0;
}

int launch_sv_round(const DevCrt &t, int V, const uint32_t *bitsL, const uint32_t *bitsR, size_t nplanes, const uint64_t *eqB, size_t ldeq, size_t pair0, size_t npairs, uint32_t K,
                    const Fq3Const *mu_pow, const uint64_t *coef, unsigned char *EB, int32_t *part, int32_t *tot, uint64_t *tp, const uint64_t *gpart, uint64_t *out,
                    hipStream_t s, hipEvent_t gpart_ready, const uint64_t *E, size_t ldE, const Fq3Const *w01) {
    const size_t wall = cdiv(nplanes, 2 * (size_t)V);
    const size_t wpairs = pair0 >= wall ? 0 : (wall - pair0 < npairs ? wall - pair0 : npairs);
    if (!sv_shape_ok(V, npairs, K) || (pair0 * V) % 256) return -1;
    const size_t ldeb = sv_ldeb(npairs);
    const bool split = E != nullptr;
    const u32 NT = split ? 2u : 3u;
    if (split) {
        (void)hipMemsetAsync(EB + 24 * ldeb, 0, 8 * ldeb, s);
        hipLaunchKernelGGL(k_sv_pack_eq, dim3((unsigned)cdiv(ldeb / 16 * 3, 256)), dim3(256), 0, s, E + pair0, ldE, npairs, ldeb, V, EB, 1);
    } else
    hipLaunchKernelGGL(k_sv_pack_eq, dim3((unsigned)cdiv(ldeb / 16 * 6, 256)), dim3(256), 0, s, eqB + 2 * pair0, ldeq, npairs, ldeb, V, EB, 0);
    SvGemmArgs a;
    a.bits[0] = bitsL; a.bits[1] = bitsR;
    a.ktiles = (K + 15) / 16;
    a.nsides = 2;
    a.rd = 24;
    a.rows = 16 * a.ktiles + 1;
    a.nw = sv_npad(nplanes) / 32;
    a.EB = EB; a.ldeb = ldeb;
    a.nsuper = (u32)cdiv(wpairs * V, 256);
    a.super0 = (u32)(pair0 * V / 256);
    a.eb_mod = 0;
    const u32 chunks = sv_chunks(V, a.nsuper, K);
    a.super_per_chunk = (u32)cdiv(a.nsuper, chunks);
    a.part = part;
    const u32 grid = 48 * a.ktiles / (u32)sv_waves(V) * chunks;
    if (split) {
        if (V == 1) launch_gemm_pg<1, 0, 2>(a, grid, s);
        else if (V == 2) launch_gemm_pg<2, 0, 2>(a, grid, s);
        else launch_gemm_pg<4, 0, 2>(a, grid, s);
    } else
    if (V == 1) launch_gemm_pg<1, 0>(a, grid, s);
    else if (V == 2) launch_gemm_pg<2, 0>(a, grid, s);
    else launch_gemm_pg<4, 0>(a, grid, s);
    const size_t words = sv_tot_words(V, K) / 3 * NT;
    hipLaunchKernelGGL(k_sv_sum, dim3((unsigned)cdiv(words / 4, 256)), dim3(256), 0, s, part, words, chunks, tot);
    const u32 npr = (u32)sv_num_pairs(V);
    const Fq3Const wz = {{0, 0, 0}}, w0 = split ? w01[0] : wz, w1 = split ? w01[1] : wz;
    if (t.nu2p40) hipLaunchKernelGGL((k_sv_finish1<true>), dim3(2 * K * 24), dim3(128), 0, s, t, tot, npr, K, a.ktiles, coef, mu_pow, tp, NT, w0, w1);
    else hipLaunchKernelGGL((k_sv_finish1<false>), dim3(2 * K * 24), dim3(128), 0, s, t, tot, npr, K, a.ktiles, coef, mu_pow, tp, NT, w0, w1);
    if (gpart_ready) (void)hipStreamWaitEvent(s, gpart_ready, 0);
    hipLaunchKernelGGL(k_sv_finish2, dim3(1), dim3(1024), 0, s, tp, K, gpart, out);
    return 0;
}

__global__ void __launch_bounds__(256) k_sv_vs_finish(const int32_t *tot, u32 K, u32 ktiles, u64 *out) {
    const u32 o = blockIdx.x * 256 + threadIdx.x;
    if (o >= K * 72) return;
    const u32 q = o % 3, c = (o / 3) % 24, k = o / 72;
    const u32 grp = c * ktiles + k / 16, krow = k & 15;
    __int128 v = 0;
#pragma unroll
    for (int h = 0; h < 2; h++) {
        const int32_t *base = tot + ((size_t)grp * 4 + (h ? 2 : 0)) * 768;
        for (u32 u = 0; u < 8; u++) {
            const u32 bp = 24 * h + 8 * q + u;
            v += (__int128)base[(bp >> 4) * 256 + ((bp & 15) + 16 * (krow >> 2)) * 4 + (krow & 3)] << (8 * u);
        }
    }
    out[o] = fq_from_s128((u64)v, (int64_t)(v >> 64));
}
size_t sv_vs_part_words(size_t, uint32_t K) { return sv_tot_words(1, K) / 2 * sv_max_chunks(1, K, 1); }
size_t sv_vs_tot_words(uint32_t K) { return sv_tot_words(1, K) / 2; }
int launch_sv_vs(const uint32_t *bits, size_t n, const uint64_t *eq, size_t ldeq, uint32_t K, unsigned char *EB, int32_t *part, int32_t *tot, uint64_t *out, hipStream_t s) {
    static_assert(sv_pair(1, 0).s == 1 && sv_pair(1, 0).b == 1 && sv_pair(1, 2).s == 2 && sv_pair(1, 2).b == 2, "single pairs of V = 1");
    const size_t npairs = n / 2;
    if ((n & 1) || !sv_shape_ok(1, npairs, K)) return -1;
    const size_t ldeb = sv_ldeb(npairs);
    hipLaunchKernelGGL(k_sv_pack_eq, dim3((unsigned)cdiv(ldeb / 16 * 6, 256)), dim3(256), 0, s, eq, ldeq, npairs, ldeb, 1, EB, 0);
    SvGemmArgs a;
    a.bits[0] = bits; a.bits[1] = bits;
    a.ktiles = (K + 15) / 16;
    a.nsides = 1;
    a.rd = 24;
    a.rows = 16 * a.ktiles + 1;
    a.nw = sv_npad(n) / 32;
    a.EB = EB; a.ldeb = ldeb;
    a.nsuper = (u32)cdiv(npairs, 256);
    a.super0 = 0;
    a.eb_mod = 0;
    const u32 chunks = sv_chunks_n(1, a.nsuper, K, 1);
    a.super_per_chunk = (u32)cdiv(a.nsuper, chunks);
    a.part = part;
    hipLaunchKernelGGL((k_sv_gemm<1, 0, 3, true>), dim3(24 * a.ktiles / (u32)sv_waves(1) * chunks), dim3(64 * sv_waves(1)), 0, s, a);
    const size_t words = sv_vs_tot_words(K);
    hipLaunchKernelGGL(k_sv_sum, dim3((unsigned)cdiv(words / 4, 256)), dim3(256), 0, s, part, words, chunks, tot);
    hipLaunchKernelGGL(k_sv_vs_finish, dim3((unsigned)cdiv((size_t)K * 72, 256)), dim3(256), 0, s, tot, K, a.ktiles, out);
    return 0;
}
size_t sv_vs_max_blocks(uint32_t) { return 256; }
size_t sv_vs_blocks_part_words(uint32_t nblocks, uint32_t K) { return sv_vs_tot_words(K) * nblocks; }
int launch_sv_vs_blocks(const uint32_t *bits, size_t n, const uint64_t *eq_lo, size_t ldeq, uint32_t J, uint32_t K, unsigned char *EB, int32_t *part, hipStream_t s) {
    if (J < 10 || J > 24 || (n & (((size_t)1 << J) - 1)) || n == 0) return -1;
    const size_t bs = (size_t)1 << J, nblocks = n / bs, lo_pairs = bs / 2;
    if (nblocks > sv_vs_max_blocks(K) || !sv_shape_ok(1, n / 2, K)) return -1;
    const size_t ldeb = sv_ldeb(lo_pairs);
    hipLaunchKernelGGL(k_sv_pack_eq, dim3((unsigned)cdiv(ldeb / 16 * 6, 256)), dim3(256), 0, s, eq_lo, ldeq, lo_pairs, ldeb, 1, EB, 0);
    SvGemmArgs a;
    a.bits[0] = bits; a.bits[1] = bits;
    a.ktiles = (K + 15) / 16;
    a.nsides = 1;
    a.rd = 24;
    a.rows = 16 * a.ktiles + 1;
    a.nw = sv_npad(n) / 32;
    a.EB = EB; a.ldeb = ldeb;
    a.nsuper = (u32)(n / 512);
    a.super0 = 0;
    a.eb_mod = (u32)(bs / 512);
    a.super_per_chunk = a.eb_mod;
    a.part = part;
    hipLaunchKernelGGL((k_sv_gemm<1, 0, 3, true>), dim3(24 * a.ktiles / (u32)sv_waves(1) * (u32)nblocks), dim3(64 * sv_waves(1)), 0, s, a);
    return 0;
}
template <bool NU>
__global__ void __launch_bounds__(64) k_sv_vs_combine(DevCrt t, const int32_t *part, u32 nblocks, size_t words, const u64 *wts, u32 K, u32 ktiles, u64 *out) {
    const u32 o = blockIdx.x, lane = threadIdx.x;
    const u32 c = o % 24, k = o / 24;
    const u32 grp = c * ktiles + k / 16, krow = k & 15;
    Fq3 acc = fq3_zero();
    for (u32 b = lane; b < nblocks; b += 64) {
        const int32_t *tot = part + (size_t)b * words;
        u64 tq[3];
#pragma unroll
        for (u32 q = 0; q < 3; q++) {
            __int128 v = 0;
#pragma unroll
            for (int h = 0; h < 2; h++) {
                const int32_t *base = tot + ((size_t)grp * 4 + (h ? 2 : 0)) * 768;
#pragma unroll
                for (u32 u = 0; u < 8; u++) {
                    const u32 bp = 24 * h + 8 * q + u;
                    v += (__int128)base[(bp >> 4) * 256 + ((bp & 15) + 16 * (krow >> 2)) * 4 + (krow & 3)] << (8 * u);
                }
            }
            tq[q] = fq_from_s128((u64)v, (int64_t)(v >> 64));
        }
        acc = fq3_add(acc, fq3_mul<NU>(fq3_make(tq[0], tq[1], tq[2]), fq3_make(wts[3 * b], wts[3 * b + 1], wts[3 * b + 2]), t.nu));
    }
#pragma unroll
    for (int off = 32; off > 0; off >>= 1)
#pragma unroll
        for (int q = 0; q < 3; q++) acc.c[q] = fq_add(acc.c[q], __shfl_down(acc.c[q], off, 64));
    if (lane == 0) { out[(size_t)o * 3] = acc.c[0]; out[(size_t)o * 3 + 1] = acc.c[1]; out[(size_t)o * 3 + 2] = acc.c[2]; }
}
void launch_sv_vs_combine(const DevCrt &t, const int32_t *part, uint32_t nblocks, const uint64_t *wts, uint32_t K, uint64_t *out, hipStream_t s) {
    const u32 ktiles = (K + 15) / 16;
    const size_t words = sv_vs_tot_words(K);
    if (t.nu2p40) hipLaunchKernelGGL((k_sv_vs_combine<true>), dim3(K * 24), dim3(64), 0, s, t, part, nblocks, words, wts, K, ktiles, out);
    else hipLaunchKernelGGL((k_sv_vs_combine<false>), dim3(K * 24), dim3(64), 0, s, t, part, nblocks, words, wts, K, ktiles, out);
}
}
```

Measured before the change: 60.98 steps/s.

## Overlap fold setup on side stream, fuse fix and sv finish kernels

Moves the mu-power upload and the eq builds into fold prepare on a second lane stream, and pre-packs the round-1 split eq operand there. The fix_special launches are merged into one segmented kernel, and the sv_sum reduction is folded into a sliced finish1 kernel. Host coefficient computation in gemm_round now runs after the GEMM stage is launched, and eq pair-sum is fused with packing. The aim is to cut launch count and serialization on the main stream, at the cost of more cross-stream dependencies and staging-buffer bookkeeping.

```diff
diff --git a/latticefold_amd/csrc/lf_capi.cpp b/latticefold_amd/csrc/lf_capi.cpp
--- a/latticefold_amd/csrc/lf_capi.cpp
+++ b/latticefold_amd/csrc/lf_capi.cpp
@@ -700,17 +700,19 @@
     return LF_OK;
 }
 
-int build_eq_dev(lf_ctx *c, const Fq3 *pt, u32 nv, u64 *eq_dev) {
+int build_eq_dev(lf_ctx *c, const Fq3 *pt, u32 nv, u64 *eq_dev, hipStream_t st) {
+    const bool side = st && st != c->stream();
+    if (!st) st = c->stream();
     Fq3Const *rd;
-    RET(c->tbuf("eq_point", 64, &rd));
+    RET(c->tbuf(side ? "eq_point_side" : "eq_point", 64, &rd));
     std::vector<Fq3Const> h(nv);
     for (u32 i = 0; i < nv; i++) h[i] = f3c(pt[i]);
-    RET(c->h2d_small(rd, h.data(), nv * sizeof(Fq3Const)));
+    RET(c->h2d_small(rd, h.data(), nv * sizeof(Fq3Const), st));
     if (nv >= 6) {
         u64 *scr;
-        RET(c->tbuf("eq_scratch", build_eq_scratch_words(nv), &scr));
-        launch_build_eq2(c->dcrt, rd, nv, scr, eq_dev, c->stream());
-    } else launch_build_eq(c->dcrt, rd, nv, eq_dev, c->stream());
+        RET(c->tbuf(side ? "eq_scratch_side" : "eq_scratch", build_eq_scratch_words(nv), &scr));
+        launch_build_eq2(c->dcrt, rd, nv, scr, eq_dev, st);
+    } else launch_build_eq(c->dcrt, rd, nv, eq_dev, st);
     return LF_OK;
 }
 static int build_eq_api(lf_ctx *c, const uint64_t *point, unsigned nv, uint64_t *out, Origin org) {
diff --git a/latticefold_amd/csrc/lf_ctx.h b/latticefold_amd/csrc/lf_ctx.h
--- a/latticefold_amd/csrc/lf_ctx.h
+++ b/latticefold_amd/csrc/lf_ctx.h
@@ -179,24 +179,29 @@
 
     unsigned char *stage[LF_NLANES] = {nullptr, nullptr, nullptr};
     size_t stage_off[LF_NLANES] = {0, 0, 0};
+    hipStream_t stage_side[LF_NLANES] = {nullptr, nullptr, nullptr};
     static constexpr size_t STAGE_BYTES = (size_t)1 << 20;
-    int h2d_small(void *dst, const void *src, size_t bytes) {
+    int h2d_small(void *dst, const void *src, size_t bytes, hipStream_t st = nullptr) {
+        if (!st) st = stream();
         unsigned char *&ring = stage[t_lane];
         if (!ring && hipHostMalloc((void **)&ring, STAGE_BYTES, hipHostMallocDefault) != hipSuccess) { ring = nullptr; return LF_ERR_HIP; }
         const size_t need = (bytes + 63) & ~(size_t)63;
         if (need > STAGE_BYTES) {
-            HIPCHK(hipMemcpyAsync(dst, src, bytes, hipMemcpyHostToDevice, stream()));
-            HIPCHK(hipStreamSynchronize(stream()));
+            HIPCHK(hipMemcpyAsync(dst, src, bytes, hipMemcpyHostToDevice, st));
+            HIPCHK(hipStreamSynchronize(st));
             return LF_OK;
         }
         if (stage_off[t_lane] + need > STAGE_BYTES) {
             HIPCHK(hipStreamSynchronize(stream()));
+            if (stage_side[t_lane]) HIPCHK(hipStreamSynchronize(stage_side[t_lane]));
+            stage_side[t_lane] = nullptr;
             stage_off[t_lane] = 0;
         }
+        if (st != stream()) stage_side[t_lane] = st;
         unsigned char *slot = ring + stage_off[t_lane];
         stage_off[t_lane] += need;
         memcpy(slot, src, bytes);
-        HIPCHK(hipMemcpyAsync(dst, slot, bytes, hipMemcpyHostToDevice, stream()));
+        HIPCHK(hipMemcpyAsync(dst, slot, bytes, hipMemcpyHostToDevice, st));
         return LF_OK;
     }
     TailMail *tail_mail = nullptr;
@@ -246,7 +251,7 @@
 #pragma GCC visibility push(hidden)
 Fq3Const f3c(Fq3 a);
 bool shard_keep(const lf_ctx *c, int kind, size_t n);
-int build_eq_dev(lf_ctx *c, const Fq3 *pt, u32 nv, u64 *eq_dev);
+int build_eq_dev(lf_ctx *c, const Fq3 *pt, u32 nv, u64 *eq_dev, hipStream_t st = nullptr);
 int exchange_modsum_dev(lf_ctx *c, u64 *inout_dev, size_t words);
 int down_small(lf_ctx *c, const u64 *dsrc, size_t words, u64 *host);
 void shard_slice(const lf_ctx *c, size_t n, size_t *i0, size_t *cnt);
@@ -334,11 +339,11 @@
     u64 *theta() const { return proof + (size_t)P.s * (deg + 1) * 24; }
     u64 *eta() const { return theta() + (size_t)K2 * 72; }
     int powers_alpha_zeta();
-    int powers_mu();
+    int powers_mu(hipStream_t st = nullptr);
     int prepare_buffers();
     int side_mz(int sd, hipStream_t st, u64 *zb, const char *zaos_name, size_t zc_lo, size_t zc_hi, size_t g_r0 = 0, size_t g_rcnt = (size_t)-1);
     void first_tables();
-    void fix_special(u32 round, Fq3Const r, u64 *dst, hipStream_t sg);
+    void fix_special(u32 round, Fq3Const r, u64 *dst, hipStream_t sg, bool eqb_on_sg = false);
     void set_tables(u64 *dst, size_t nn);
     int eval_buffers();
     int gather_q(hipStream_t s1f);
diff --git a/latticefold_amd/csrc/lf_fold.cpp b/latticefold_amd/csrc/lf_fold.cpp
--- a/latticefold_amd/csrc/lf_fold.cpp
+++ b/latticefold_amd/csrc/lf_fold.cpp
@@ -107,10 +107,11 @@
     RET(upload_consts(c, "c_ap", a_pow, &d_ap));
     return upload_consts(c, "c_zp", z_pow, &d_zp);
 }
-int FoldStep::powers_mu() {
+int FoldStep::powers_mu(hipStream_t st) {
     std::vector<Fq3Const> mu_pow((size_t)K2 * 3);
     for (u32 i = 0; i < K2; i++) lfs::powers(hv, mu[i], 3, [&](u32 d, const Fq3 &pw) { mu_pow[(size_t)i * 3 + d] = f3c(pw); });
-    return upload_consts(c, "c_mu", mu_pow, &d_mu);
+    RET(c->tbuf("c_mu", mu_pow.size() + 8, &d_mu));
+    return c->h2d_small(d_mu, mu_pow.data(), mu_pow.size() * sizeof(Fq3Const), st);
 }
 int FoldStep::prepare_buffers() {
     RET(c->tbuf("fold_G1", 24 * m, &G[0]));
@@ -136,21 +137,26 @@
     a.eqL = dst; a.eqR = dst + 3 * nn; a.eqB = dst + 6 * nn; a.G1 = dst + 9 * nn; a.G2 = dst + 33 * nn;
     a.ld = nn; a.n = nn;
 }
-void FoldStep::fix_special(u32 round, Fq3Const r, u64 *dst, hipStream_t sg) {
+void FoldStep::fix_special(u32 round, Fq3Const r, u64 *dst, hipStream_t sg, bool eqb_on_sg) {
     const size_t nn = a.n / 2;
+    const bool together = eqb_on_sg || sg == c->stream();
+    if (round > 2 && together) {
+        launch_fix_many(c->dcrt, a.eqL, a.ld, dst, nn, a.n, 19, r, sg);
+        return;
+    }
+    FixSegs fs;
     if (round == 2) {
-        launch_fix_many(c->dcrt, a.eqL, a.ld, dst, nn, a.n, 1, r, sg);
-        launch_fix_many(c->dcrt, a.eqR, a.ld, dst + 3 * nn, nn, a.n, 1, r, sg);
-        launch_fix_many(c->dcrt, a.eqB, a.ld, dst + 6 * nn, nn, a.n, 1, r, c->stream());
-        launch_fix_many(c->dcrt, a.G1, a.ld, dst + 9 * nn, nn, a.n, 8, r, sg);
-        launch_fix_many(c->dcrt, a.G2, a.ld, dst + 33 * nn, nn, a.n, 8, r, sg);
-    } else if (sg != c->stream()) {
-        launch_fix_many(c->dcrt, a.eqL, a.ld, dst, nn, a.n, 2, r, sg);
-        launch_fix_many(c->dcrt, a.eqB, a.ld, dst + 6 * nn, nn, a.n, 1, r, c->stream());
-        launch_fix_many(c->dcrt, a.G1, a.ld, dst + 9 * nn, nn, a.n, 16, r, sg);
+        fs.add(a.eqL, dst, 1);
+        fs.add(a.eqR, dst + 3 * nn, 1);
+        if (together) fs.add(a.eqB, dst + 6 * nn, 1);
+        fs.add(a.G1, dst + 9 * nn, 8);
+        fs.add(a.G2, dst + 33 * nn, 8);
     } else {
-        launch_fix_many(c->dcrt, a.eqL, a.ld, dst, nn, a.n, 19, r, c->stream());
-    }
+        fs.add(a.eqL, dst, 2);
+        fs.add(a.G1, dst + 9 * nn, 16);
+    }
+    launch_fix_segs(c->dcrt, fs, a.ld, nn, a.n, r, sg);
+    if (!together) launch_fix_many(c->dcrt, a.eqB, a.ld, dst + 6 * nn, nn, a.n, 1, r, c->stream());
 }
 int FoldStep::eval_buffers() {
     u64 *fsm;
@@ -236,7 +242,7 @@
     u64 *svE[3] = {nullptr, nullptr, nullptr}, *svE_rest = nullptr;
     u32 svE_level = 1;
     lfs::SplitCoef<GoldV> sp{};
-    bool split_now = false;
+    bool split_now = false, eb1_packed = false;
     const u64 *Er = nullptr;
     u64 *F[2] = {nullptr, nullptr}, *partial = nullptr, *od = nullptr, *od_host = nullptr, *od_shard = nullptr, *d_lut = nullptr;
     u32 *sv_bits[2] = {nullptr, nullptr};
@@ -251,6 +257,13 @@
     void svE_ensure(u32 l) {
         for (; svE_level < l; svE_level++)
             launch_eq_pairsum(svE_ptr(svE_level), m >> svE_level, m >> (svE_level + 1), svE_ptr(svE_level + 1), m >> (svE_level + 1), c->stream());
+    }
+    bool sv_enabled() const {
+        return !c->tn.force_exchange && !c->tn.fold_no_sv && (Gw == 1 || !c->tn.shard_plain_rounds) && N <= m && (N & 3) == 0 && !c->tn.fold_tab_r1;
+    }
+    bool gemm_round_ok(u32 round, size_t pcnt, size_t p0) const {
+        return sv_enabled() && (int)round <= c->tn.sv_rounds && round <= 3 && pcnt >= c->tn.sv_min && sv_shape_ok(1 << (round - 1), pcnt, K) &&
+               (p0 * ((size_t)1 << (round - 1))) % 256 == 0;
     }
     int prepare(), rounds_begin(), tail_handoff(u32 round, bool *done), fix_tables(u32 round, u64 *dst, bool *gathered), choose_producer(u32 round);
     void decide_split(u32 round);
@@ -287,15 +300,23 @@
     }
     { HostTimer ht(c); lfs::draw_mu_beta<GoldV>(tr, K2, P.s, mu, beta); }
     TL_MARK(" fold challenges");
-    RET(powers_mu());
-    RET(build_eq_dev(c, beta.data(), P.s, eqb));
+    hipStream_t se = (t_lane == 0 && Gw == 1) ? c->st_lane[1] : c->stream();
+    RET(powers_mu(se));
+    RET(build_eq_dev(c, beta.data(), P.s, eqb, se));
     sv_split = !c->tn.fold_sv_no_split && P.s >= 4 && m >= 256;
     if (sv_split) {
         RET(c->tbuf("fold_svE1", 3 * (m / 2), &svE[0]));
         RET(c->tbuf("fold_svE2", 3 * (m / 4), &svE[1]));
         RET(c->tbuf("fold_svE3", 3 * (m / 8), &svE[2]));
-        RET(build_eq_dev(c, beta.data() + 1, P.s - 1, svE[0]));
-    }
+        RET(build_eq_dev(c, beta.data() + 1, P.s - 1, svE[0], se));
+        if (se != c->stream() && gemm_round_ok(1, m / 2, 0)) {
+            unsigned char *sveb;
+            RET(c->tbuf("sv_eb", sv_eb_bytes(m / 2), &sveb));
+            launch_sv_pack_split(1, svE[0], m / 2, m / 2, sveb, se);
+            eb1_packed = true;
+        }
+    }
+    RET(c->join(se, c->stream()));
     fr_split = sv_split && c->sh_world == 1 && c->dcrt.nu2p40 && !c->tn.fold_rounds_no_split;
     if (fr_split) RET(c->tbuf("fold_svE_rest", 3 * (m / 8) + 64, &svE_rest));
     LF_TRACE(c, "fold prepare");
@@ -319,7 +340,7 @@
     c->fold_split_mask = 0;
     sv_two_streams = t_lane == 0 && Gw == 1;
     sv_g_stream = c->stream();
-    use_sv = !c->tn.force_exchange && !c->tn.fold_no_sv && (Gw == 1 || !c->tn.shard_plain_rounds) && N <= m && (N & 3) == 0 && !c->tn.fold_tab_r1;
+    use_sv = sv_enabled();
     return LF_OK;
 }
 int FoldB2::tail_handoff(u32 round, bool *done) {
@@ -337,10 +358,9 @@
     const size_t nn = a.n / 2;
     const bool handover = sharded && !shard_keep(c, 1, nn);
     hipStream_t sg = c->stream();
-    if (use_sv && sv_two_streams && !sharded && (int)round <= c->tn.sv_rounds && round <= 3 && nn / 2 >= c->tn.sv_min && sv_shape_ok(1 << (round - 1), nn / 2, K))
-        sg = c->st_lane[1];
+    if (sv_two_streams && !sharded && gemm_round_ok(round, nn / 2, 0)) sg = c->st_lane[1];
     sv_g_stream = sg;
-    if (!sharded) { fix_special(round, r, dst, sg); return LF_OK; }
+    if (!sharded) { fix_special(round, r, dst, sg, sg != c->stream() && sv_split); return LF_OK; }
     const size_t j0 = gr * (nn / Gw), jc = nn / Gw;
     if (round == 2) {
         launch_fix_many(c->dcrt, a.eqL + 2 * j0, a.ld, dst + j0, nn, 2 * jc, 1, r, sg);
@@ -403,51 +423,56 @@
 }
 int FoldB2::gemm_round(u32 round) {
     const int svV = 1 << (round - 1);
-    std::vector<Fq3> W((size_t)svV), Cf;
-    lfs::eq_weights(hv, pt.data(), round - 1, W.data());
-    lfs::sv_coef(hv, svV, W.data(), sv_num_pairs(svV), [&](int i) { return sv_pair(svV, i); }, Cf);
     u64 *d_coef, *gtmp, *svtp;
     unsigned char *sveb;
-    int32_t *svpart, *svtot;
-    RET(c->tbuf("sv_coef", Cf.size() * 3 + 8, &d_coef));
+    int32_t *svpart;
+    RET(c->tbuf("sv_coef", (size_t)sv_num_pairs(svV) * 12 + 8, &d_coef));
     RET(c->tbuf("sv_gtmp", 128, &gtmp));
     RET(c->tbuf("sv_tp", sv_tp_words(K), &svtp));
     RET(c->tbuf("sv_eb", sv_eb_bytes(a.pcnt), &sveb));
     RET(c->tbuf("sv_part", sv_part_words(svV, a.pcnt, K), &svpart));
-    RET(c->tbuf("sv_tot", sv_tot_words(svV, K), &svtot));
-    RET(c->h2d_small(d_coef, Cf.data(), Cf.size() * sizeof(Fq3)));
     if (!sv_bits[0])
         for (int sd = 0; sd < 2; sd++) {
             if (S[sd].sv_bits) { sv_bits[sd] = S[sd].sv_bits; continue; }
             RET(c->tbuf(sd ? "sv_bits_R" : "sv_bits_L", sv_bits_words(N, K), &sv_bits[sd]));
             launch_sv_bits(S[sd].planes, N, N, K, sv_bits[sd], c->stream());
         }
+    const u64 *Ei = nullptr, *Eprev = nullptr;
+    size_t ldE = 0;
+    if (sv_split) {
+        Ei = svE[round - 1]; ldE = m >> round;
+        if (round >= 2 && svE_level == round - 1 && a.p0 == 0 && a.pcnt == ldE) { Eprev = svE[round - 2]; svE_level = round; }
+        else svE_ensure(round);
+    }
+    Fq3Const w01[2] = {};
+    auto sv_launch = [&](int stages, hipEvent_t g_ready) {
+        return launch_sv_round(c->dcrt, svV, sv_bits[0], sv_bits[1], N, a.eqB, a.ld, a.p0, a.pcnt, K, d_mu, d_coef, sveb, svpart, svtp, gtmp, od, c->stream(), g_ready,
+                               Ei, ldE, w01, Eprev, m >> (round - 1), round == 1 && eb1_packed && sv_split, stages);
+    };
     hipStream_t sg = round == 1 ? (sv_two_streams && !sharded ? c->st_lane[1] : c->stream()) : sv_g_stream;
     if (round == 1) RET(c->fork(c->stream(), sg));
+    if (sv_launch(1, nullptr) != 0) return LF_ERR_UNSUPPORTED;
     launch_fold_round_g(c->dcrt, a, partial, gtmp, sg);
     hipEvent_t g_ready = nullptr;
     if (sg != c->stream() && !(g_ready = c->join_mark(sg))) return LF_ERR_HIP;
-    const u64 *Ei = nullptr;
-    size_t ldE = 0;
-    Fq3Const w01[2] = {};
+    std::vector<Fq3> W((size_t)svV), Cf;
+    lfs::eq_weights(hv, pt.data(), round - 1, W.data());
+    lfs::sv_coef(hv, svV, W.data(), sv_num_pairs(svV), [&](int i) { return sv_pair(svV, i); }, Cf);
+    if (Cf.size() != (size_t)sv_num_pairs(svV) * 4) return LF_ERR_INVALID;
+    RET(c->h2d_small(d_coef, Cf.data(), Cf.size() * sizeof(Fq3)));
     if (sv_split) {
         const Fq3 ci = lfs::eq_prefix(hv, beta.data(), pt.data(), round), bi = beta[round - 1];
         w01[0] = f3c(hv.ext_mul(ci, fq3_sub(fq3_one(), bi)));
         w01[1] = f3c(hv.ext_mul(ci, bi));
-        svE_ensure(round);
-        Ei = svE[round - 1]; ldE = m >> round;
-    }
-    if (launch_sv_round(c->dcrt, svV, sv_bits[0], sv_bits[1], N, a.eqB, a.ld, a.p0, a.pcnt, K, d_mu, d_coef, sveb, svpart, svtot, svtp, gtmp, od, c->stream(), g_ready,
-                        Ei, ldE, w01) != 0)
-        return LF_ERR_UNSUPPORTED;
+    }
+    if (sv_launch(2, g_ready) != 0) return LF_ERR_UNSUPPORTED;
     c->sv_round_mask |= 1u << (round - 1);
     return LF_OK;
 }
 int FoldB2::dispatch(u32 round) {
     const int32_t *pL = S[0].planes, *pR = S[1].planes;
     hipStream_t st = c->stream();
-    if (use_sv && (int)round <= c->tn.sv_rounds && round <= 3 && a.pcnt >= c->tn.sv_min && sv_shape_ok(1 << (round - 1), a.pcnt, K) && (a.p0 * ((size_t)1 << (round - 1))) % 256 == 0)
-        return gemm_round(round);
+    if (use_sv && gemm_round_ok(round, a.pcnt, a.p0)) return gemm_round(round);
     if ((round == 2 || (round == 1 && c->tn.fold_tab_r1)) && a.pcnt >= c->tn.tab_min) {
         std::vector<u64> poly;
         fold_tab_poly(hv, round, round == 2 ? pt[0] : fq3_zero(), poly);
diff --git a/latticefold_amd/csrc/lf_kernels.h b/latticefold_amd/csrc/lf_kernels.h
--- a/latticefold_amd/csrc/lf_kernels.h
+++ b/latticefold_amd/csrc/lf_kernels.h
@@ -81,6 +81,15 @@
                         long long *tot, u64 *out, hipStream_t s, bool y_packed = false, u32 nb_out = 0, u32 b0 = 0);
 int launch_dot_pack_y(const u64 *X, const u64 *Y, size_t ldy, u32 nb, size_t n, unsigned char *YB, hipStream_t s);
 void launch_vs_combine(const u64 *vs , u32 K, u64 *v , hipStream_t s);
+constexpr int FIX_MAX_SEGS = 5;
+struct FixSegs {
+    const u64 *in[FIX_MAX_SEGS];
+    u64 *out[FIX_MAX_SEGS];
+    u32 rows3[FIX_MAX_SEGS];
+    u32 n = 0;
+    void add(const u64 *i, u64 *o, u32 r) { in[n] = i; out[n] = o; rows3[n] = r; n++; }
+};
+void launch_fix_segs(const DevCrt &t, const FixSegs &sg, size_t ld_in, size_t ld_out, size_t n_in, Fq3Const r, hipStream_t s);
 void launch_fix_final(const DevCrt &t, const u64 *in , u32 rows3, Fq3Const r, u64 *out , hipStream_t s);
 
 struct LinCombDesc {
diff --git a/latticefold_amd/csrc/lf_kernels.hip b/latticefold_amd/csrc/lf_kernels.hip
--- a/latticefold_amd/csrc/lf_kernels.hip
+++ b/latticefold_amd/csrc/lf_kernels.hip
@@ -744,6 +744,43 @@
     size_t n_out = n_in / 2;
     LF_LAUNCH(k_fix, t.nu2p40, dim3(cdiv(n_out, 256), rows3), dim3(256), s, t, in, ld_in, out, ld_out, n_out, r);
 }
+struct FixSegArgs {
+    const u64 *in[FIX_MAX_SEGS];
+    u64 *out[FIX_MAX_SEGS];
+    u32 end[FIX_MAX_SEGS];
+};
+template <bool NU>
+__global__ void __launch_bounds__(256) k_fix_segs(DevCrt t, FixSegArgs a, size_t ld_in, size_t ld_out, size_t n_out, Fq3Const r) {
+    const size_t j = (size_t)blockIdx.x * 256 + threadIdx.x;
+    if (j >= n_out) return;
+    const u32 y = blockIdx.y;
+    const u64 *p = a.in[0];
+    u64 *q = a.out[0];
+    u32 row = y;
+#pragma unroll
+    for (int i = 1; i < FIX_MAX_SEGS; i++)
+        if (y >= a.end[i - 1]) { p = a.in[i]; q = a.out[i]; row = y - a.end[i - 1]; }
+    p += (size_t)row * 3 * ld_in;
+    q += (size_t)row * 3 * ld_out;
+    const Fq3 rr = fq3_make(r.c[0], r.c[1], r.c[2]);
+    const ulonglong2 a0 = *(const ulonglong2 *)(p + 2 * j), a1 = *(const ulonglong2 *)(p + ld_in + 2 * j), a2 = *(const ulonglong2 *)(p + 2 * ld_in + 2 * j);
+    const Fq3 v0 = fq3_make(a0.x, a1.x, a2.x), v1 = fq3_make(a0.y, a1.y, a2.y);
+    const Fq3 res = fq3_add(v0, M3<NU>(fq3_sub(v1, v0), rr, t.nu));
+    q[j] = res.c[0]; q[ld_out + j] = res.c[1]; q[2 * ld_out + j] = res.c[2];
+}
+void launch_fix_segs(const DevCrt &t, const FixSegs &sg, size_t ld_in, size_t ld_out, size_t n_in, Fq3Const r, hipStream_t s) {
+    const size_t n_out = n_in / 2;
+    FixSegArgs a;
+    u32 rows = 0;
+    for (u32 i = 0; i < (u32)FIX_MAX_SEGS; i++) {
+        const u32 k = i < sg.n ? i : sg.n - 1;
+        a.in[i] = sg.in[k]; a.out[i] = sg.out[k];
+        if (i < sg.n) rows += sg.rows3[i];
+        a.end[i] = rows;
+    }
+    if (!rows || !n_out) return;
+    LF_LAUNCH(k_fix_segs, t.nu2p40, dim3(cdiv(n_out, 256), rows), dim3(256), s, t, a, ld_in, ld_out, n_out, r);
+}
 
 template <bool NU>
 __global__ void __launch_bounds__(256) k_fix_final(DevCrt t, const u64 *in, u32 rows3, Fq3Const r, u64 *out) {
diff --git a/latticefold_amd/csrc/lf_sv_rounds.h b/latticefold_amd/csrc/lf_sv_rounds.h
--- a/latticefold_amd/csrc/lf_sv_rounds.h
+++ b/latticefold_amd/csrc/lf_sv_rounds.h
@@ -48,9 +48,13 @@
 struct DevCrt;
 struct Fq3Const;
 int launch_sv_round(const DevCrt &t, int V, const uint32_t *bitsL, const uint32_t *bitsR, size_t nplanes, const uint64_t *eqB, size_t ldeq, size_t pair0, size_t npairs, uint32_t K,
-                    const Fq3Const *mu_pow, const uint64_t *coef, unsigned char *EB, int32_t *part, int32_t *tot, uint64_t *tp, const uint64_t *gpart, uint64_t *out,
+                    const Fq3Const *mu_pow, const uint64_t *coef, unsigned char *EB, int32_t *part, uint64_t *tp, const uint64_t *gpart, uint64_t *out,
                     hipStream_t s, hipEvent_t gpart_ready = nullptr,
-                    const uint64_t *E = nullptr, size_t ldE = 0, const Fq3Const *w01 = nullptr);
+                    const uint64_t *E = nullptr, size_t ldE = 0, const Fq3Const *w01 = nullptr,
+                    const uint64_t *Eprev = nullptr, size_t ldEprev = 0,
+                    bool eb_ready = false,
+                    int stages = 3);
+void launch_sv_pack_split(int V, const uint64_t *E, size_t ldE, size_t npairs, unsigned char *EB, hipStream_t s);
 size_t sv_vs_part_words(size_t n, uint32_t K);
 size_t sv_vs_tot_words(uint32_t K);
 int launch_sv_vs(const uint32_t *bits, size_t n, const uint64_t *eq, size_t ldeq, uint32_t K, unsigned char *EB, int32_t *part, int32_t *tot, uint64_t *out, hipStream_t s);
diff --git a/latticefold_amd/csrc/lf_sv_rounds.hip b/latticefold_amd/csrc/lf_sv_rounds.hip
--- a/latticefold_amd/csrc/lf_sv_rounds.hip
+++ b/latticefold_amd/csrc/lf_sv_rounds.hip
@@ -52,16 +52,25 @@
 
 __host__ __device__ constexpr int sv_slot_pair(int V, int j, int q) { return (j / (4 / V)) * (16 / V) + (j % (4 / V)) + (4 / V) * q; }
 
-__global__ void __launch_bounds__(256) k_sv_pack_eq(const u64 *eq, size_t ld, size_t npairs, size_t ldeb, int V, unsigned char *EB, int single) {
+template <int MODE>
+__global__ void __launch_bounds__(256) k_sv_pack_eq(const u64 *eq, size_t ld, size_t npairs, size_t ldeb, int V, unsigned char *EB, u64 *eo, size_t ldo) {
     const size_t gid = (size_t)blockIdx.x * 256 + threadIdx.x, groups = ldeb / 16;
-    if (gid >= groups * (single ? 3 : 6)) return;
+    if (gid >= groups * (MODE ? 3 : 6)) return;
     const u32 qh = (u32)(gid / groups), q = qh % 3, h = qh / 3;
     const size_t p0 = (gid % groups) * 16;
     u64 w[16];
 #pragma unroll
     for (int t = 0; t < 16; t++) {
         const size_t pr = p0 + (size_t)sv_slot_pair(V, t >> 2, t & 3);
-        const u64 e = pr < npairs ? (single ? eq[(size_t)q * ld + pr] : eq[(size_t)q * ld + 2 * pr + h]) : 0;
+        u64 e = 0;
+        if (pr < npairs) {
+            if constexpr (MODE == 2) {
+                const ulonglong2 a = *(const ulonglong2 *)(eq + (size_t)q * ld + 2 * pr);
+                e = fq_add(a.x, a.y);
+                eo[(size_t)q * ldo + pr] = e;
+            } else
+                e = MODE ? eq[(size_t)q * ld + pr] : eq[(size_t)q * ld + 2 * pr + h];
+        }
         u64 sb = e + 0x8080808080808080ull;
         if (sb < e) sb += 0xFFFFFFFFull;
         w[t] = sb ^ 0x8080808080808080ull;
@@ -73,6 +82,14 @@
         for (int t = 0; t < 16; t++) o[t >> 2] |= (u32)((w[t] >> (8 * u)) & 0xFF) << (8 * (t & 3));
         *(uint4 *)(EB + (size_t)(24 * h + 8 * q + u) * ldeb + p0) = make_uint4(o[0], o[1], o[2], o[3]);
     }
+    if constexpr (MODE != 0)
+        for (u32 r = 24 + 3 * q; r < 27 + 3 * q && r < 32; r++) *(uint4 *)(EB + (size_t)r * ldeb + p0) = make_uint4(0, 0, 0, 0);
+}
+static void launch_pack_eq(int mode, const u64 *eq, size_t ld, size_t npairs, size_t ldeb, int V, unsigned char *EB, u64 *eo, size_t ldo, hipStream_t s) {
+    const dim3 grid((unsigned)cdiv(ldeb / 16 * (mode ? 3 : 6), 256)), block(256);
+    if (mode == 0) hipLaunchKernelGGL(k_sv_pack_eq<0>, grid, block, 0, s, eq, ld, npairs, ldeb, V, EB, eo, ldo);
+    else if (mode == 1) hipLaunchKernelGGL(k_sv_pack_eq<1>, grid, block, 0, s, eq, ld, npairs, ldeb, V, EB, eo, ldo);
+    else hipLaunchKernelGGL(k_sv_pack_eq<2>, grid, block, 0, s, eq, ld, npairs, ldeb, V, EB, eo, ldo);
 }
 
 __device__ __forceinline__ u32 sv_full(u32 x) {
@@ -217,19 +234,38 @@
     *(v4i *)(tot + i) = s;
 }
 
+constexpr u32 SV_FPS = 64, SV_FPST = 3 * 64 + 4;
+static u32 sv_finish_slices(int V) { return ((u32)sv_num_pairs(V) + SV_FPS - 1) / SV_FPS; }
 template <bool NU>
-__global__ void __launch_bounds__(128) k_sv_finish1(DevCrt t, const int32_t *tot, u32 npr, u32 K, u32 ktiles, const u64 *coef, const Fq3Const *mu_pow, u64 *tp, u32 nt, Fq3Const w0,
-                                                    Fq3Const w1) {
-    const u32 T = blockIdx.x, c = T % 24, k = (T / 24) % K, side = T / (24 * K);
-    const u32 grp = (side * 24 + c) * ktiles + k / 16, krow = k & 15;
-    __shared__ u64 sm[15][128];
-    const u32 pi = threadIdx.x;
+__global__ void __launch_bounds__(256) k_sv_finish1(DevCrt t, const int32_t *part, size_t words, u32 chunks, u32 npr, u32 K, u32 ktiles, const u64 *coef, const Fq3Const *mu_pow,
+                                                    u64 *tp, u32 nt, Fq3Const w0, Fq3Const w1) {
+    const u32 g = blockIdx.x & 3, grp = blockIdx.x >> 2, slice = blockIdx.y;
+    const u32 kt = grp % ktiles, c = (grp / ktiles) % 24, side = grp / (ktiles * 24), k0 = 16 * kt + 4 * g;
+    if (k0 >= K) return;
+    __shared__ __attribute__((aligned(16))) unsigned char raw[SV_FPS * SV_FPST * 4];
+    int32_t *cells = (int32_t *)raw;
+    u64(*sm)[256] = (u64(*)[256])raw;
+    static_assert(sizeof(raw) >= 15 * 256 * 8, "the reduction reuses the cells' LDS");
+    const u32 tid = threadIdx.x, pi0 = slice * SV_FPS, pn = npr - pi0 < SV_FPS ? npr - pi0 : SV_FPS;
+    for (u32 it = tid; it < pn * nt * 16; it += 256) {
+        const u32 l16 = it & 15, tile = (it >> 4) % nt, pl = it / (16 * nt);
+        v4i s = v4i{0, 0, 0, 0};
+        if (nt == 3 || tile == 0 || l16 < 8) {
+            const int32_t *src = part + ((size_t)grp * npr + pi0 + pl) * (nt * 256) + tile * 256 + (16 * g + l16) * 4;
+#pragma unroll 4
+            for (u32 ch = 0; ch < chunks; ch++) s += *(const v4i *)(src + (size_t)ch * words);
+        }
+        *(v4i *)(cells + pl * SV_FPST + tile * 64 + l16 * 4) = s;
+    }
+    __syncthreads();
+    const u32 pl = tid >> 2, kk = tid & 3, k = k0 + kk;
     Fq3 P[5];
 #pragma unroll
     for (int e = 0; e < 5; e++) P[e] = fq3_zero();
-    if (pi < npr) {
-        const int32_t *base = tot + ((size_t)grp * npr + pi) * (nt * 256);
-        auto cell = [&](u32 bp) { return (long long)base[(bp >> 4) * 256 + ((bp & 15) + 16 * (krow >> 2)) * 4 + (krow & 3)]; };
+    if (pl < pn && k < K) {
+        const u32 pi = pi0 + pl;
+        const int32_t *base = cells + pl * SV_FPST + kk;
+        auto cell = [&](u32 bp) { return (long long)base[(bp >> 4) * 64 + (bp & 15) * 4]; };
         Fq3 M[2];
 #pragma unroll
         for (int h = 0; h < 2; h++)
@@ -254,33 +290,35 @@
             P[e + 1] = fq3_add(P[e + 1], fq3_mul<NU>(C, dM, t.nu));
         }
     }
+    __syncthreads();
 #pragma unroll
     for (int e = 0; e < 5; e++)
 #pragma unroll
-        for (int q = 0; q < 3; q++) sm[3 * e + q][threadIdx.x] = P[e].c[q];
-    __syncthreads();
-    if (threadIdx.x < 15) {
-        u64 s = 0;
-        for (u32 i = 0; i < 128; i++) s = fq_add(s, sm[threadIdx.x][i]);
-        sm[threadIdx.x][0] = s;
-    }
-    __syncthreads();
-    if (threadIdx.x < 5) {
-        const u32 e = threadIdx.x;
-        const Fq3Const mc = mu_pow[(side * K + k) * 3 + c / 8];
-        const Fq3 r = fq3_mul<NU>(fq3_make(mc.c[0], mc.c[1], mc.c[2]), fq3_make(sm[3 * e][0], sm[3 * e + 1][0], sm[3 * e + 2][0]), t.nu);
-#pragma unroll
-        for (int q = 0; q < 3; q++) tp[((size_t)T * 5 + e) * 3 + q] = fq_canon(r.c[q]);
-    }
-}
-__global__ void __launch_bounds__(1024) k_sv_finish2(const u64 *tp, u32 K, const u64 *gpart, u64 *out) {
+        for (int q = 0; q < 3; q++) sm[3 * e + q][tid] = P[e].c[q];
+    __syncthreads();
+    u64 s = 0;
+    if (tid < 60)
+        for (u32 i = 0; i < SV_FPS; i++) s = fq_add(s, sm[tid % 15][4 * i + tid / 15]);
+    __syncthreads();
+    if (tid < 60) sm[tid % 15][tid / 15] = s;
+    __syncthreads();
+    if (tid < 20 && k0 + tid / 5 < K) {
+        const u32 e = tid % 5, kq = tid / 5, kx = k0 + kq;
+        const size_t T = ((size_t)side * K + kx) * 24 + c;
+        const Fq3Const mc = mu_pow[(side * K + kx) * 3 + c / 8];
+        const Fq3 r = fq3_mul<NU>(fq3_make(mc.c[0], mc.c[1], mc.c[2]), fq3_make(sm[3 * e][kq], sm[3 * e + 1][kq], sm[3 * e + 2][kq]), t.nu);
+#pragma unroll
+        for (int q = 0; q < 3; q++) tp[(((size_t)slice * 2 * K * 24 + T) * 5 + e) * 3 + q] = fq_canon(r.c[q]);
+    }
+}
+__global__ void __launch_bounds__(1024) k_sv_finish2(const u64 *tp, u32 K, u32 nsl, const u64 *gpart, u64 *out) {
     __shared__ u64 sm[8][128];
     const u32 i = threadIdx.x & 127, j = threadIdx.x >> 7;
     const u32 X = i / 24, slot = (i % 24) / 3, q = i % 3;
     u64 v = 0;
     if (i < 120) {
         u64 co[5] = {0, 0, 0, 0, 0};
-        for (u32 sk = j; sk < 2 * K; sk += 8)
+        for (u32 sk = j; sk < 2 * K * nsl; sk += 8)
             for (u32 d = 0; d < 3; d++) {
                 const u64 *p = tp + ((size_t)(sk * 24 + 8 * d + slot) * 5) * 3 + q;
 #pragma unroll
@@ -332,7 +370,7 @@
     return per_chunk >= 256 ? 1 : 256 / per_chunk;
 }
 size_t sv_part_words(int V, size_t, uint32_t K) { return sv_tot_words(V, K) * sv_max_chunks(V, K, 2); }
-size_t sv_tp_words(uint32_t K) { return (size_t)2 * K * 24 * 15; }
+size_t sv_tp_words(uint32_t K) { return (size_t)2 * K * 24 * 15 * sv_finish_slices(4); }
 
 size_t sv_tot_words_rd(uint32_t rd, int V, uint32_t K) { return (size_t)2 * rd * ((K + 15) / 16) * sv_num_pairs(V) * 768; }
 size_t sv_part_words_rd(uint32_t rd, int V, uint32_t K) { return sv_tot_words_rd(rd, V, K) * sv_max_chunks(V, K, 2, rd); }
@@ -364,20 +402,25 @@
     return 0;
 }
 
+void launch_sv_pack_split(int V, const uint64_t *E, size_t ldE, size_t npairs, unsigned char *EB, hipStream_t s) {
+    launch_pack_eq(1, E, ldE, npairs, sv_ldeb(npairs), V, EB, nullptr, 0, s);
+}
 int launch_sv_round(const DevCrt &t, int V, const uint32_t *bitsL, const uint32_t *bitsR, size_t nplanes, const uint64_t *eqB, size_t ldeq, size_t pair0, size_t npairs, uint32_t K,
-                    const Fq3Const *mu_pow, const uint64_t *coef, unsigned char *EB, int32_t *part, int32_t *tot, uint64_t *tp, const uint64_t *gpart, uint64_t *out,
-                    hipStream_t s, hipEvent_t gpart_ready, const uint64_t *E, size_t ldE, const Fq3Const *w01) {
+                    const Fq3Const *mu_pow, const uint64_t *coef, unsigned char *EB, int32_t *part, uint64_t *tp, const uint64_t *gpart, uint64_t *out,
+                    hipStream_t s, hipEvent_t gpart_ready, const uint64_t *E, size_t ldE, const Fq3Const *w01, const uint64_t *Eprev, size_t ldEprev, bool eb_ready, int stages) {
     const size_t wall = cdiv(nplanes, 2 * (size_t)V);
     const size_t wpairs = pair0 >= wall ? 0 : (wall - pair0 < npairs ? wall - pair0 : npairs);
     if (!sv_shape_ok(V, npairs, K) || (pair0 * V) % 256) return -1;
     const size_t ldeb = sv_ldeb(npairs);
     const bool split = E != nullptr;
     const u32 NT = split ? 2u : 3u;
-    if (split) {
-        (void)hipMemsetAsync(EB + 24 * ldeb, 0, 8 * ldeb, s);
-        hipLaunchKernelGGL(k_sv_pack_eq, dim3((unsigned)cdiv(ldeb / 16 * 3, 256)), dim3(256), 0, s, E + pair0, ldE, npairs, ldeb, V, EB, 1);
+    if (Eprev && (!split || pair0 || npairs > ldE)) return -1;
+    if (eb_ready || !(stages & 1)) {
+    } else if (split) {
+        if (Eprev) launch_pack_eq(2, Eprev, ldEprev, npairs, ldeb, V, EB, const_cast<uint64_t *>(E), ldE, s);
+        else launch_pack_eq(1, E + pair0, ldE, npairs, ldeb, V, EB, nullptr, 0, s);
     } else
-    hipLaunchKernelGGL(k_sv_pack_eq, dim3((unsigned)cdiv(ldeb / 16 * 6, 256)), dim3(256), 0, s, eqB + 2 * pair0, ldeq, npairs, ldeb, V, EB, 0);
+        launch_pack_eq(0, eqB + 2 * pair0, ldeq, npairs, ldeb, V, EB, nullptr, 0, s);
     SvGemmArgs a;
     a.bits[0] = bitsL; a.bits[1] = bitsR;
     a.ktiles = (K + 15) / 16;
@@ -393,7 +436,8 @@
     a.super_per_chunk = (u32)cdiv(a.nsuper, chunks);
     a.part = part;
     const u32 grid = 48 * a.ktiles / (u32)sv_waves(V) * chunks;
-    if (split) {
+    if (!(stages & 1)) {
+    } else if (split) {
         if (V == 1) launch_gemm_pg<1, 0, 2>(a, grid, s);
         else if (V == 2) launch_gemm_pg<2, 0, 2>(a, grid, s);
         else launch_gemm_pg<4, 0, 2>(a, grid, s);
@@ -401,14 +445,15 @@
     if (V == 1) launch_gemm_pg<1, 0>(a, grid, s);
     else if (V == 2) launch_gemm_pg<2, 0>(a, grid, s);
     else launch_gemm_pg<4, 0>(a, grid, s);
+    if (!(stages & 2)) return 0;
     const size_t words = sv_tot_words(V, K) / 3 * NT;
-    hipLaunchKernelGGL(k_sv_sum, dim3((unsigned)cdiv(words / 4, 256)), dim3(256), 0, s, part, words, chunks, tot);
-    const u32 npr = (u32)sv_num_pairs(V);
+    const u32 npr = (u32)sv_num_pairs(V), nsl = sv_finish_slices(V);
     const Fq3Const wz = {{0, 0, 0}}, w0 = split ? w01[0] : wz, w1 = split ? w01[1] : wz;
-    if (t.nu2p40) hipLaunchKernelGGL((k_sv_finish1<true>), dim3(2 * K * 24), dim3(128), 0, s, t, tot, npr, K, a.ktiles, coef, mu_pow, tp, NT, w0, w1);
-    else hipLaunchKernelGGL((k_sv_finish1<false>), dim3(2 * K * 24), dim3(128), 0, s, t, tot, npr, K, a.ktiles, coef, mu_pow, tp, NT, w0, w1);
+    const dim3 fgrid(48 * a.ktiles * 4, nsl);
+    if (t.nu2p40) hipLaunchKernelGGL((k_sv_finish1<true>), fgrid, dim3(256), 0, s, t, part, words, chunks, npr, K, a.ktiles, coef, mu_pow, tp, NT, w0, w1);
+    else hipLaunchKernelGGL((k_sv_finish1<false>), fgrid, dim3(256), 0, s, t, part, words, chunks, npr, K, a.ktiles, coef, mu_pow, tp, NT, w0, w1);
     if (gpart_ready) (void)hipStreamWaitEvent(s, gpart_ready, 0);
-    hipLaunchKernelGGL(k_sv_finish2, dim3(1), dim3(1024), 0, s, tp, K, gpart, out);
+    hipLaunchKernelGGL(k_sv_finish2, dim3(1), dim3(1024), 0, s, tp, K, nsl, gpart, out);
     return 0;
 }
 
@@ -435,7 +480,7 @@
     const size_t npairs = n / 2;
     if ((n & 1) || !sv_shape_ok(1, npairs, K)) return -1;
     const size_t ldeb = sv_ldeb(npairs);
-    hipLaunchKernelGGL(k_sv_pack_eq, dim3((unsigned)cdiv(ldeb / 16 * 6, 256)), dim3(256), 0, s, eq, ldeq, npairs, ldeb, 1, EB, 0);
+    launch_pack_eq(0, eq, ldeq, npairs, ldeb, 1, EB, nullptr, 0, s);
     SvGemmArgs a;
     a.bits[0] = bits; a.bits[1] = bits;
     a.ktiles = (K + 15) / 16;
@@ -463,7 +508,7 @@
     const size_t bs = (size_t)1 << J, nblocks = n / bs, lo_pairs = bs / 2;
     if (nblocks > sv_vs_max_blocks(K) || !sv_shape_ok(1, n / 2, K)) return -1;
     const size_t ldeb = sv_ldeb(lo_pairs);
-    hipLaunchKernelGGL(k_sv_pack_eq, dim3((unsigned)cdiv(ldeb / 16 * 6, 256)), dim3(256), 0, s, eq_lo, ldeq, lo_pairs, ldeb, 1, EB, 0);
+    launch_pack_eq(0, eq_lo, ldeq, lo_pairs, ldeb, 1, EB, nullptr, 0, s);
     SvGemmArgs a;
     a.bits[0] = bits; a.bits[1] = bits;
     a.ktiles = (K + 15) / 16;
```

New measurement: 61.02 steps/s, median of 3. About the same (+0.1%).
